# PaddlePaddle/Anakin

Measured on AMD Instinct MI355X. Metric: ResNet50 INT8 images/sec + p50 latency @ batch 1/8, 1×MI355X, higher is better.
Workload: dtype int8

## Files before the change

anakin_amd/build.py:

```python
import os
import subprocess
import sys

HERE = os.path.dirname(os.path.abspath(__file__))
CSRC = os.path.join(HERE, "csrc")
LIB = os.path.join(HERE, "libsaber_mi355x.so")
SOURCES = ["conv_igemm.hip", "elementwise.hip", "fc_small.hip", "conv1x1_chain.hip", "conv_chain_coop.hip", "conv_stage_coop.hip", "stage_xcd.hip", "conv1x1_gpool.hip", "conv3x3_b3h.hip", "conv1x1_pw.hip", "conv1x1_pwk.hip", "conv_stem_f32.hip", "fc_f32_splitk.hip", "conv_dw3x3.hip", "conv_group3x3.hip", "conv_sep.hip", "conv_ir.hip", "conv_fire.hip", "deconv.hip"] + \
    ["api_%s.hip" % n for n in ("conv", "select", "autotune", "ops", "chain", "sep", "ir", "fire", "deconv", "stage", "net", "net_optimize", "net_autotune", "capture", "gemm", "streams")] + \
    ["igemm_m%d_e%d.hip" % me for me in [(0, 0), (0, 1), (0, 2), (0, 3), (0, 4), (1, 0), (1, 1), (1, 2), (1, 3), (2, 3), (3, 3)]] + \
    ["igemm_dma_m%d_e%d.hip" % me for me in [(0, 0), (0, 1), (0, 2), (0, 3), (0, 4), (2, 3)]] + \
    ["halo_e%d.hip" % e for e in range(4)] + ["img_e%d.hip" % e for e in (0, 1, 3)] + ["stem_e%d.hip" % e for e in range(4)] + ["stem_pool.hip"]
FLAGS = ["--offload-arch=gfx950", "-O3", "-std=c++17", "-fPIC", "-ffp-contract=off", "-fno-fast-math",
         "-Wno-unused-result", "-mllvm", "-amdgpu-mfma-vgpr-form"]


def _stale(obj, deps):
    if not os.path.exists(obj):
        return True
    t = os.path.getmtime(obj)
    return any(os.path.getmtime(d) > t for d in deps)


def build(force=False, verbose=False):
    hipcc = os.environ.get("HIPCC", "/opt/rocm/bin/hipcc")
    objdir = os.path.join(HERE, "build")
    os.makedirs(objdir, exist_ok=True)
    import glob
    headers = sorted(glob.glob(os.path.join(CSRC, "*.h"))) + [os.path.join(HERE, "..", "include", "saber_hip.h")]
    objs = []
    procs = []
    for src in SOURCES:
        sp = os.path.join(CSRC, src)
        obj = os.path.join(objdir, src.replace(".hip", ".o"))
        objs.append(obj)
        deps = [h for h in headers if src.startswith("api_") or os.path.basename(h) != "api_internal.h"]
        if force or _stale(obj, [sp] + deps):
            cmd = [hipcc] + FLAGS + ["-c", sp, "-o", obj]
            if verbose:
                print(" ".join(cmd))
            procs.append((src, subprocess.Popen(cmd)))
# ... 35 lines not shown
```

anakin_amd/csrc/api_chain.hip:

```cpp
#include "api_internal.h"

enum : unsigned { CK_1X1 = 1, CK_3X3 = 2, CK_HEAD = 4, CK_PAIR = 8, CK_LED = CK_3X3 | CK_HEAD, CK_ANY = 15 };
static unsigned chain_kind(const saber_hip_chain* ch) { return !ch->c3 ? CK_1X1 : (ch->b2 ? CK_PAIR : (ch->b ? CK_3X3 : CK_HEAD)); }
static const struct { int c1; unsigned kinds; ChainForm f; } chain_forms[] = {
    {64, CK_ANY,            {4, 4, 4, 1, 1, CS_BASE, false}},
    {64, CK_ANY,            {2, 2, 4, 1, 1, CS_BASE, false}},
    {128, CK_1X1 | CK_LED,  {2, 2, 4, 1, 1, CS_BASE, false}},
    {128, CK_1X1 | CK_LED,  {1, 1, 4, 1, 1, CS_BASE, false}},
    {128, CK_1X1 | CK_LED,  {6, 2, 8, 1, 1, CS_W8, false}},
    {128, CK_1X1 | CK_LED,  {5, 1, 8, 1, 1, CS_W8, false}},
    {256, CK_1X1 | CK_LED,  {1, 1, 4, 1, 1, CS_BASE, false}},
    {256, CK_1X1,           {9, 1, 4, 2, 1, CS_SPLIT, false}},
    {256, CK_1X1,           {11, 1, 8, 2, 1, CS_SPLIT8, false}},
    {256, CK_LED,           {3, 1, 8, 1, 1, CS_W8, false}},
    {256, CK_3X3,           {7, 1, 8, 1, 2, CS_COOP2, true}},
    {256, CK_3X3,           {15, 2, 8, 1, 4, CS_COOP4, true}},
    {512, CK_1X1,           {1, 1, 4, 1, 1, CS_BASE, false}},
    {512, CK_1X1,           {9, 1, 4, 2, 1, CS_SPLIT, false}},
};
static void for_each_chain_form(const saber_hip_chain* ch, const std::function<void(const ChainForm&)>& fn) {
    for (const auto& r : chain_forms)
        if (r.c1 == ch->c1 && (r.kinds & chain_kind(ch))) fn(r.f);
}
static ChainForm chain_form_where(const saber_hip_chain* ch, const std::function<bool(const ChainForm& row, const ChainForm& found)>& take) {
    ChainForm f;
    for_each_chain_form(ch, [&](const ChainForm& c) { if (take(c, f)) f = c; });
    return f;
}
ChainForm chain_form(const saber_hip_chain* ch, int code) { return chain_form_where(ch, [&](const ChainForm& c, const ChainForm&) { return c.code == code; }); }
ChainForm chain_form_default(const saber_hip_chain* ch) { return chain_form_where(ch, [](const ChainForm&, const ChainForm& f) { return !f.code; }); }
ChainForm chain_form_plain(const saber_hip_chain* ch) { return chain_form_where(ch, [](const ChainForm& c, const ChainForm&) { return !c.placement; }); }
bool chain_form_valid(const saber_hip_chain* ch, int code) {
    const ChainForm f = chain_form(ch, code);
    return f.code && ch->d_stream[f.stream].p && (f.coop != 4 || ch->stage1);
}
std::string chain_form_name(const saber_hip_chain* ch) {
    const ChainForm& f = ch->form;
    const std::string c = std::to_string(ch->c1), w8 = f.waves == 8 && f.coop == 1 ? "_w8" : "";
    if (!ch->c3) return "chain1x1_c" + c + "_px" + std::to_string(16 * f.rows) + (f.split == 2 ? "_split2" : "") + w8;
    return std::string("conv3x3+") + (ch->b2 ? "conv1x1+pair1x1_c" : (ch->b ? "chain1x1_c" : "conv1x1_c")) + c + "_" + std::to_string(f.rows) + "x16" + w8 +
           (f.coop == 2 ? "_coop2" : "") + (f.coop == 4 ? "_coop4" : "");
}
void for_each_chain_candidate(const saber_hip_chain* ch, bool shared_device, const std::function<void(const ChainForm&)>& fn) {
    for_each_chain_form(ch, [&](const ChainForm& c) { if (!(shared_device && c.placement) && chain_form_valid(ch, c.code)) fn(c); });
}

static bool chain_1x1(const saber_hip_conv* o, bool sub_res_ok = false) {
    const saber_hip_conv_desc& d = o->d;
    return o->is_i8 && o->weights_set && !o->gpool && o->algo == ALGO_IGEMM_I8 && o->epi == EPI_I8_CONV && d.kh == 1 && d.kw == 1 &&
           d.stride_h == 1 && d.stride_w == 1 && d.pad_h == 0 && d.pad_w == 0 && d.group == 1 && !o->pair_k2 &&
           !o->pool_fused && !o->pool2 && !o->pre_quant && !o->pre_pad && o->c_eff == d.c && d.act_negative_slope == 0.f &&
           d.in_layout == SABER_HIP_NHWC && d.out_layout == SABER_HIP_NHWC && (d.res_stride <= 1 || sub_res_ok);
}
static void pack_chain_params(const saber_hip_conv* o, size_t chunks_pad, std::vector<uint8_t>& out) {
    const int K = o->d.k;
    out.assign(chunks_pad * 16, 0);
    for (int k4 = 0; k4 < K / 4; ++k4) {
        float* f = (float*)(out.data() + (size_t)k4 * 48);
        int* ip = (int*)(out.data() + (size_t)k4 * 48 + 32);
        for (int r = 0; r < 4; ++r) {
            const int k = k4 * 4 + r;
            f[r] = o->scale_host.empty() ? 1.f : o->scale_host[k];
            f[4 + r] = (o->has_bias && !o->bias_p_host.empty()) ? o->bias_p_host[k] : 0.f;
            ip[r] = o->comp_host.empty() ? 0 : o->comp_host[k];
        }
    }
}
// ... 471 lines not shown
        if (rc != SABER_HIP_OK) {
            delete ch;
            return rc;
        }
    }
    *out = ch;
    return SABER_HIP_OK;
}
int saber_hip_conv2d_chain_create(saber_hip_conv_t* a, saber_hip_conv_t* b, saber_hip_chain_t** out) {
    if (!b) return fail(SABER_HIP_INVALID_VALUE, "null argument");
    return chain_build(nullptr, a, b, out);
}
int saber_hip_conv2d_chain_create3(saber_hip_conv_t* conv3x3, saber_hip_conv_t* a, saber_hip_conv_t* b, saber_hip_chain_t** out) {
    if (!conv3x3) return fail(SABER_HIP_INVALID_VALUE, "null argument");
    return chain_build(conv3x3, a, b, out);
}
int saber_hip_conv2d_chain_create3_pair(saber_hip_conv_t* conv3x3, saber_hip_conv_t* a, saber_hip_conv_t* pair_a, saber_hip_conv_t* pair_b,
                                        saber_hip_chain_t** out) {
    if (!conv3x3 || !pair_a || !pair_b) return fail(SABER_HIP_INVALID_VALUE, "null argument");
    return chain_build(conv3x3, a, pair_a, out, pair_b);
}
void saber_hip_conv2d_chain_destroy(saber_hip_chain_t* ch) { delete ch; }
int saber_hip_conv2d_chain_set_tile(saber_hip_chain_t* ch, int tn) {
    if (!ch) return fail(SABER_HIP_INVALID_VALUE, "null argument");
    if (!chain_form_valid(ch, tn)) return fail(SABER_HIP_INVALID_VALUE, "chain: no kernel form with that code for this chain");
    ch->form = chain_form(ch, tn);
    return SABER_HIP_OK;
}
int saber_hip_conv2d_chain_get_tile(const saber_hip_chain_t* ch) { return ch ? ch->form.code : 0; }
int saber_hip_conv2d_chain_run(saber_hip_chain_t* ch, const void* x, const void* res, void* y_a, void* y_b,
                               saber_hip_stream_t stream) {
    return saber_hip_conv2d_chain_run3(ch, x, res, y_a, y_b, nullptr, stream);
}
int saber_hip_conv2d_chain_run3(saber_hip_chain_t* ch, const void* x, const void* res, void* y_a, void* y_b, void* y_c,
                                saber_hip_stream_t stream) {
    if (g_capture) return capture_unsupported("saber_hip_conv2d_chain_run (saber_hip_net_optimize forms chains itself)");
    if (!ch || !x || !res || !y_a || (ch->b && !y_b) || (ch->b2 && !y_c)) return fail(SABER_HIP_INVALID_VALUE, "null argument");
    const saber_hip_conv *a = ch->a, *b = ch->b;
    ChainKArgs k;
    std::memset(&k, 0, sizeof k);
    k.x = x; k.res = res;
    const ChainForm f = ch->form;
    k.wstream = ch->d_stream[f.stream].p;
    k.prm1 = ch->d_prm1.p;
    k.prm2 = ch->d_prm2.p;
    k.y1 = y_a; k.y2 = y_b;
    k.M = a->d.n * a->oh * a->ow;
    k.in_u8 = a->x_dtype == DT_U8;
    k.relu1 = a->d.act == SABER_HIP_ACT_RELU;
    k.res_relu = a->d.res_act == SABER_HIP_ACT_RELU;
    k.coeff_conv = a->d.coeff_conv; k.scale_conv = ch->scale_conv; k.coeff_res = a->d.coeff_res; k.scale_res = a->d.scale_res;
    if (b) {
        k.relu2 = b->d.act == SABER_HIP_ACT_RELU;
        k.out_u8_2 = b->d.out_dtype == SABER_HIP_U8;
    }
    if (ch->b2) {
        k.y2b = y_c;
        k.k2_split = b->d.k;
        k.relu2b = ch->b2->d.act == SABER_HIP_ACT_RELU;
        k.out_u8_2b = ch->b2->d.out_dtype == SABER_HIP_U8;
    }
    if (ch->c3) {
        k.prm0 = ch->d_prm0.p;
        k.zero = zero_page();
        if (!k.zero) return fail(SABER_HIP_RUNTIME_ERROR, "chain: zero page");
        k.N = a->d.n; k.H = a->d.h; k.W = a->d.w;
        k.tiles_x = (k.W + 15) / 16;
        k.tiles_per_img = k.tiles_x * ((k.H + f.rows - 1) / f.rows);
        k.mg_tiles_x = div_magic(k.tiles_x);
        k.mg_tpi = div_magic(k.tiles_per_img);
        k.in0_u8 = ch->c3->x_dtype == DT_U8;
        k.relu0 = ch->c3->d.act == SABER_HIP_ACT_RELU;
        k.s0 = ch->c3->d.stride_h;
        k.H0 = ch->c3->d.h; k.W0 = ch->c3->d.w;
        if (a->d.res_stride > 1) { k.res_sub = a->d.res_stride; k.res_H = a->d.res_h; k.res_W = a->d.res_w; }
    }
    if (f.coop == 4) {
        const int rc = stage_run(ch->stage1, x, res, &y_a, &y_b, (hipStream_t)stream);
        if (rc != SABER_HIP_OK) ch->form = chain_form_plain(ch);
        return rc;
    }
    if (f.coop == 2) {
        if (*(volatile unsigned*)ch->h_coop_err) {
            *(volatile unsigned*)ch->h_coop_err = 0u;
            ch->form = chain_form_plain(ch);
            return fail(SABER_HIP_RUNTIME_ERROR, "cooperative chain: an earlier launch's workgroup pairs did not share an XCD or timed out at their "
                        "barrier (its outputs are not valid); the chain now runs the single-workgroup form");
        }
        const CoopKArgs ck{k, ch->d_coop_ctr.p, ch->d_coop_xch.p, ch->d_coop_xcc.p, ch->h_coop_err, ch->coop_tiles};
        HIP_TRY(launch_conv_chain_coop(ck, (hipStream_t)stream));
        return SABER_HIP_OK;
    }
    HIP_TRY(launch_conv1x1_chain(k, ch->c1, ch->k1, ch->k2, f.rows, f.waves, f.split, ch->c3 ? 1 : 0, (hipStream_t)stream));
    return SABER_HIP_OK;
}
```

anakin_amd/csrc/api_internal.h:

```cpp
#pragma once
#include "../../include/saber_hip.h"
#include "kernels.h"

#include <cmath>
#include <cstdio>
#include <algorithm>
#include <cstdlib>
#include <cstring>
#include <functional>
#include <memory>
#include <mutex>
#include <string>
#include <utility>
#include <type_traits>
#include <vector>

using namespace saber_mi355x;

namespace saber_api {

extern thread_local std::string g_err;
inline int fail(int code, const std::string& msg) {
    g_err = msg;
    return code;
// ... 147 lines not shown
    bool has_bias = false, has_comp = false;
    std::string algo_name;
    int pair_k1 = 0, pair_k2 = 0, pair_relu2 = 0, pair_dtype2 = 0;
    const saber_hip_conv* pair_src_a = nullptr;
    const saber_hip_conv* pair_src_b = nullptr;
};

struct saber_hip_stem_pair {
    saber_hip_conv* stem = nullptr;
    const saber_hip_conv* a = nullptr;
    const saber_hip_conv* b = nullptr;
    DevBuf<uint8_t> d_w, d_prm;
};

enum ChainStream { CS_BASE, CS_SPLIT, CS_SPLIT8, CS_W8, CS_COOP2, CS_COOP4, CS_COUNT };
struct ChainForm {
    int code = 0;
    int rows = 0;
    int waves = 4;
    int split = 1;
    int coop = 1;
    ChainStream stream = CS_BASE;
    bool placement = false;
};

struct saber_hip_chain {
    saber_hip_conv* c3 = nullptr;
    saber_hip_conv* a = nullptr;
    saber_hip_conv* b = nullptr;
    saber_hip_conv* b2 = nullptr;
    int c1 = 0, k1 = 0, k2 = 0;
    float scale_conv = 1.f;
    std::vector<int8_t> tail_w3, tail_wa;
    ChainForm form;
    DevBuf<uint8_t> d_stream[CS_COUNT];
    DevBuf<uint8_t> d_prm0, d_prm1, d_prm2;
    DevBuf<uint8_t> d_coop_xch;
    DevBuf<uint8_t> d_stream_stage1;
    DevBuf<unsigned long long> d_coop_ctr;
    DevBuf<unsigned> d_coop_xcc;
    unsigned* h_coop_err = nullptr;
    int coop_tiles = 0;
    struct saber_hip_chain_stage* stage1 = nullptr;
    ~saber_hip_chain();
};

struct saber_hip_chain_stage {
    std::vector<saber_hip_chain*> chains;
    saber_hip_chain* tail = nullptr;
    DevBuf<uint8_t> d_tail_stream;
    const saber_hip_conv* head_a = nullptr;
    const saber_hip_conv* head_b = nullptr;
    DevBuf<uint8_t> d_head_stream, d_head_prm1, d_head_prm2;
    DevBuf<saber_mi355x::StageBlk> d_blk;
    DevBuf<unsigned long long> d_grp_ctr, d_img_ctr;
    DevBuf<uint8_t> d_xch;
    DevBuf<unsigned> d_xcc;
    unsigned* h_err = nullptr;
    int c1 = 0, n = 0, h = 0, w = 0, tiles_x = 0, tiles_per_img = 0;
    bool per_image = false;
    ~saber_hip_chain_stage() {
        if (h_err) (void)hipHostFree(h_err);
    }
};

struct saber_hip_sep {
// ... 112 lines not shown
        owner = true;
        return hipSuccess;
    }
    ~ColdScope() {
        if (owner) g_cold = nullptr;
    }
};

}

namespace saber_api {
enum OpKind { OP_CONV, OP_CONV_PAIR, OP_FC, OP_QUANT, OP_DEQUANT, OP_TRANSPOSE_IN, OP_ELT_I8, OP_ELT_F32, OP_POOL_I8, OP_POOL_F32, OP_POOL_F32_I8, OP_FC_Q, OP_SOFTMAX, OP_RELU_F32, OP_ACT_F32, OP_CONCAT, OP_DECONV };
enum Launch { LAUNCH_NONE, LAUNCH_OWN, LAUNCH_CHAIN, LAUNCH_CHAIN3, LAUNCH_STAGE, LAUNCH_STEM_PAIR, LAUNCH_SEP, LAUNCH_IR, LAUNCH_FIRE };
struct NetOp {
    OpKind kind;
    std::string name;
    saber_hip_conv* conv = nullptr;
    saber_hip_fc* fc = nullptr;
    saber_hip_deconv* deconv = nullptr;
    int in = -1, in2 = -1, out = -1, out2 = -1;
    std::vector<int> ins, cat_c;
    std::vector<float> cat_m;
    Launch launch = LAUNCH_OWN;
    int absorbed_by = -1;
    bool skip = false;
    std::string res_note;
    saber_hip_chain* chain = nullptr;
    int chain_out = -1;
    bool chain_on = false;
    saber_hip_chain* chain3 = nullptr;
    int chain3_res = -1, chain3_y1 = -1, chain3_y2 = -1;
    int chain3_y3 = -1;
    bool led_on = false;
    saber_hip_chain_stage* stage = nullptr;
    int stage_n = 0;
    bool stage_on = false;
    bool stage_name_kept = false;
    bool tail_on = false;
    int tail_of = -1;
    bool head_on = false;
    int head_of = -1;
    bool stage_y1_private = false;
    saber_hip_stem_pair* stem_pair = nullptr;
    int stem_y1 = -1, stem_y2 = -1;
    saber_hip_sep* sep = nullptr;
    int sep_out = -1;
    bool sep_on = false;
    saber_hip_ir* ir = nullptr;
    int ir_out = -1;
    bool ir_on = false;
    saber_hip_fire* fire = nullptr;
    int fire_out = -1;
    bool fire_on = false;
    int lane = 0;
    bool record = false;
    int p[16] = {0};
    float f[6] = {0};
    size_t count = 0;
};
template <typename F>
inline void op_for_each_input(const NetOp& o, F&& f) {
    if (o.kind == OP_CONCAT) {
        for (int t : o.ins) f(t);
        return;
    }
    if (o.in >= 0) f(o.in);
// ... 58 lines not shown
int sel_set(saber_hip_conv* op, const saber_api::ConvSel& s);
void sel_release_unused(saber_hip_conv* op);
void sel_name(saber_hip_conv* op);
unsigned long long sel_kernel_key(const saber_hip_conv* op, const saber_api::ConvSel& s);
int sel_launch(saber_hip_conv* op, saber_mi355x::ConvKArgs& a, hipStream_t s);
void for_each_candidate(const saber_hip_conv* op, const saber_api::ConvSel* best, const std::function<void(const saber_api::ConvSel&)>& fn);
bool dw_ok(const saber_hip_conv* op);
bool group_ok(const saber_hip_conv* op);
bool stem_ok(const saber_hip_conv* op);
bool fc_small_ok(const saber_hip_conv* op);
bool b3_tile_ok(const saber_hip_conv* op, int tile, int ks);
int dw_static_form(const saber_hip_conv* op);
int group_static_form(const saber_hip_conv* op);
constexpr long DW_STRIP_MIN_LANES = 150000;
void conv_fill_args(const saber_hip_conv* op, saber_mi355x::ConvKArgs& a, const void* x, void* y, const void* res);
int stem_pool_args(const saber_hip_conv* op, const void* x, void* y, void* workspace, hipStream_t s, saber_mi355x::ConvKArgs* a);
bool xcd_round_robin();
int split_prepare(saber_hip_conv* op);
bool img_conv_ok(const saber_hip_conv* op);
int img_conv_prepare(saber_hip_conv* op);
int pw_prepare(saber_hip_conv* op);
bool pw_eligible(const saber_hip_conv* op);
int img_conv_run(saber_hip_conv* op, const void* x, void* y, const void* res, void* y_pool, hipStream_t stream);
void img_conv_release(saber_hip_conv* op);
int net_launch(saber_hip_net* net, const NetOp& o, hipStream_t s);
bool fc_softmax_ok(const saber_hip_fc* fc, bool quantised_input = false);
int fc_run_softmax(saber_hip_fc* fc, const void* x, float* y, float* prob, void* workspace, hipStream_t s, bool quantised_input);
int fc_softmax_prepare(saber_hip_fc* fc);
int concat_check(int n_inputs, const int* channels, const float* mult, int dtype, int* row_bytes);
void net_resolve(saber_hip_net* net);
void net_drop_graph(saber_hip_net* net);
void net_set_chain_mode(saber_hip_net* net, int ia, int mode);
int net_chain_mode(const saber_hip_net* net, int ia);
void net_set_stage(saber_hip_net* net, int i0, bool on);
void net_set_head(saber_hip_net* net, int i0, bool on);
void net_set_tail(saber_hip_net* net, int i0, bool on);
ChainForm chain_form(const saber_hip_chain* ch, int code);
bool chain_form_valid(const saber_hip_chain* ch, int code);
ChainForm chain_form_default(const saber_hip_chain* ch);
ChainForm chain_form_plain(const saber_hip_chain* ch);
std::string chain_form_name(const saber_hip_chain* ch);
void for_each_chain_candidate(const saber_hip_chain* ch, bool shared_device, const std::function<void(const ChainForm&)>& fn);
bool conv_sep_ok(const saber_hip_conv* dw, const saber_hip_conv* pw, std::string* why);
bool sep_form_valid(const saber_hip_sep* sp, int code);
void for_each_sep_form(const saber_hip_sep* sp, const std::function<void(int code)>& fn);
int sep_static_form(const saber_hip_sep* sp);
void net_set_sep(saber_hip_net* net, int i, int code);
bool conv_ir_ok(const saber_hip_conv* expand, const saber_hip_conv* dw, const saber_hip_conv* project, std::string* why);
bool ir_form_valid(const saber_hip_ir* ir, int code);
void for_each_ir_form(const saber_hip_ir* ir, const std::function<void(int code)>& fn);
int ir_static_form(const saber_hip_ir* ir);
void net_set_ir(saber_hip_net* net, int i, int code);
bool conv_fire_ok(const saber_hip_conv* squeeze, const saber_hip_conv* e1, const saber_hip_conv* e3, std::string* why);
bool fire_form_valid(const saber_hip_fire* fr, int code);
void for_each_fire_form(const saber_hip_fire* fr, const std::function<void(int code)>& fn);
int fire_static_form(const saber_hip_fire* fr);
void net_set_fire(saber_hip_net* net, int i, int code);
bool deconv_form_valid(const saber_hip_deconv* op, int form);
int deconv_static_form(const saber_hip_deconv* op);
void for_each_deconv_form(const saber_hip_deconv* op, const std::function<void(int form)>& fn);
int stage_run(saber_hip_chain_stage* st, const void* x, const void* res, void* const* y1, void* const* y2, hipStream_t s, void* y_tail = nullptr,
              void* y_head = nullptr);
```

anakin_amd/csrc/api_net.hip:

```cpp
#include "api_internal.h"

#include <atomic>
static std::atomic<int> g_coop_fallbacks_total{0};

void net_drop_graph(saber_hip_net* net) {
    if (net->exec) (void)hipGraphExecDestroy(net->exec);
    if (net->graph) (void)hipGraphDestroy(net->graph);
    net->exec = nullptr;
    net->graph = nullptr;
}
int net_launch(saber_hip_net* net, const NetOp& o, hipStream_t s) {
    auto T = [&](int id) -> void* { return net->ptr(id); };
    void* ws = net->arena + net->ws_off;
    switch (o.kind) {
    case OP_CONV:
        switch (o.launch) {
        case LAUNCH_NONE: return SABER_HIP_OK;
        case LAUNCH_STAGE: {
            void* y1[saber_mi355x::STAGE4_LONG];
            void* y2[saber_mi355x::STAGE4_LONG];
            const NetOp* ops = &o;
            for (int k = 0; k < o.stage_n; ++k) {
                y1[k] = ops[3 * k].stage_y1_private ? nullptr : T(ops[3 * k].chain3_y1);
                y2[k] = T(ops[3 * k].chain3_y2);
            }
            void* const y_tail = o.tail_on ? T(ops[3 * o.stage_n].chain3_y1) : nullptr;
            const int rc = o.head_on ? stage_run(o.stage, T(ops[-1].in), nullptr, y1, y2, s, y_tail, T(o.in))
                                     : stage_run(o.stage, T(o.in), T(o.chain3_res), y1, y2, s, y_tail);
            if (rc == SABER_HIP_RUNTIME_ERROR) {
                ++net->coop_fallbacks;
                ++g_coop_fallbacks_total;
                net_set_stage(net, (int)(&o - net->ops.data()), false);
                net_drop_graph(net);
            }
            return rc;
        }
        case LAUNCH_STEM_PAIR: return saber_hip_conv2d_stem_pair_run(o.stem_pair, T(o.in), nullptr, T(o.stem_y1), T(o.stem_y2), ws, s);
        case LAUNCH_CHAIN3: {
            const int rc = saber_hip_conv2d_chain_run3(o.chain3, T(o.in), T(o.chain3_res), T(o.chain3_y1), T(o.chain3_y2), T(o.chain3_y3), s);
            if (rc == SABER_HIP_RUNTIME_ERROR) {
                ++net->coop_fallbacks;
                ++g_coop_fallbacks_total;
            }
            return rc;
        }
        case LAUNCH_CHAIN: return saber_hip_conv2d_chain_run(o.chain, T(o.in), T(o.in2), T(o.out), T(o.chain_out), s);
        case LAUNCH_SEP: return saber_hip_conv2d_sep_run(o.sep, T(o.in), nullptr, T(o.sep_out), s);
        case LAUNCH_IR: return saber_hip_conv2d_ir_run(o.ir, T(o.in), nullptr, nullptr, T(o.ir_out), s);
        case LAUNCH_FIRE: return saber_hip_conv2d_fire_run(o.fire, T(o.in), nullptr, T(o.fire_out), s);
        case LAUNCH_OWN: break;
        }
        if (o.conv->gpool) return saber_hip_conv2d_run_gpool(o.conv, T(o.in), T(o.out), T(o.in2), T(o.out2), s);
        return saber_hip_conv2d_run(o.conv, T(o.in), T(o.out), T(o.in2), ws, s);
    case OP_CONV_PAIR:
        if (o.skip) return SABER_HIP_OK;
        return saber_hip_conv2d_run_pair(o.conv, T(o.in), T(o.out), T(o.out2), s);
    case OP_FC:
        if (o.out2 >= 0) return fc_run_softmax(o.fc, T(o.in), (float*)T(o.out), (float*)T(o.out2), ws, s, false);
        return saber_hip_fc_run(o.fc, T(o.in), (float*)T(o.out), ws, s);
    case OP_QUANT:
        return saber_hip_quantize_nchw_to_nhwc(o.p[0], o.p[1], o.p[2], o.p[3], o.p[4], o.p[5], o.f[0],
                                               (const float*)T(o.in), T(o.out), s);
    case OP_DEQUANT:
        return saber_hip_dequantize_nhwc_to_nchw(o.p[0], o.p[1], o.p[2], o.p[3], o.p[4], o.f[0], T(o.in),
                                                 (float*)T(o.out), s);
    case OP_TRANSPOSE_IN:
        return saber_hip_transpose_nchw_to_nhwc_f32(o.p[0], o.p[1], o.p[2], o.p[3], o.p[4], (const float*)T(o.in),
                                                    (float*)T(o.out), s);
    case OP_ELT_I8:
        return saber_hip_eltwise_sum_i8(o.count, (const int8_t*)T(o.in), (const int8_t*)T(o.in2), o.f[0], o.f[1],
                                        o.f[2], o.f[3], o.p[0], (int8_t*)T(o.out), s);
// ... 231 lines not shown
    net->ws_off = off;
    off += (net->ws_bytes + 255) / 256 * 256;
    net->arena_bytes = off ? off : 256;
    HIP_TRY(hipMalloc((void**)&net->arena, net->arena_bytes));
    HIP_TRY(hipMemset(net->arena, 0, net->arena_bytes));
    HIP_TRY(hipStreamSynchronize(nullptr));
    net->finalized = true;
    return SABER_HIP_OK;
}
int saber_hip_net_compact_arena(saber_hip_net_t* net, const int* keep, int n_keep) {
    if (!net || !net->finalized) return fail(SABER_HIP_INVALID_VALUE, "compact_arena: net not finalized");
    const int nt = (int)net->tensor_bytes.size(), nops = (int)net->ops.size();
    for (const NetOp& o : net->ops)
        if (o.lane) return SABER_HIP_OK;
    std::vector<int> first(nt, nops), last(nt, -1), writes(nt, 0), reads(nt, 0);
    std::vector<char> pinned(nt, 0);
    for (int i = 0; i < n_keep; ++i)
        if (keep && keep[i] >= 0 && keep[i] < nt) pinned[keep[i]] = 1;
    std::vector<int> g_lo(nops), g_hi(nops);
    for (int i = 0; i < nops; ++i) g_lo[i] = g_hi[i] = i;
    auto span = [&](int i, int n) {
        const int hi = std::min(nops - 1, i + n - 1);
        int lo = i;
        for (int j = i; j <= hi; ++j) lo = std::min(lo, g_lo[j]);
        int h2 = hi;
        for (int j = i; j <= hi; ++j) h2 = std::max(h2, g_hi[j]);
        for (int j = lo; j <= h2; ++j) { g_lo[j] = std::min(g_lo[j], lo); g_hi[j] = std::max(g_hi[j], h2); }
    };
    for (int i = 0; i < nops; ++i) {
        const NetOp& o = net->ops[i];
        if (o.stage) span(i, 3 * o.stage_n + (o.stage->tail ? 2 : 0));
        if (o.stage && o.stage->head_a && i > 0) span(i - 1, 2);
        if (o.chain3) span(i, 3);
        if (o.chain) span(i, 2);
        if (o.stem_pair) span(i, 2);
        if (o.sep) span(i, 2);
        if (o.fire) span(i, 4);
        if (o.ir) span(i, 3);
        if ((o.kind == OP_FC || o.kind == OP_FC_Q) && o.out2 >= 0) span(i, 2);
    }
    for (int i = 0; i < nops; ++i) {
        const NetOp& o = net->ops[i];
        const int rd[] = {o.in, o.in2, o.chain3_res};
        const int wr[] = {o.out, o.out2, o.chain_out, o.chain3_y1, o.chain3_y2, o.chain3_y3, o.stem_y1, o.stem_y2, o.sep_out, o.ir_out, o.fire_out};
        auto touch = [&](int t) {
            if (t < 0 || t >= nt) return;
            first[t] = std::min(first[t], g_lo[i]);
            last[t] = std::max(last[t], g_hi[i]);
        };
        for (int t : rd) { touch(t); if (t >= 0 && t < nt) ++reads[t]; }
        for (size_t k = 1; k < o.ins.size(); ++k) { touch(o.ins[k]); if (o.ins[k] >= 0 && o.ins[k] < nt) ++reads[o.ins[k]]; }
        for (int t : wr) { touch(t); if (t >= 0 && t < nt) ++writes[t]; }
    }
    for (int t = 0; t < nt; ++t)
        if (net->tensor_ext[t] || !writes[t] || !reads[t] || last[t] < 0) pinned[t] = 1;
    for (int t = 0; t < nt; ++t)
        if (pinned[t]) { first[t] = -1; last[t] = nops; }
    std::vector<int> order;
    for (int t = 0; t < nt; ++t)
        if (!net->tensor_ext[t]) order.push_back(t);
    auto slot = [&](int t) { return (net->tensor_bytes[t] + 255) / 256 * 256; };
    std::stable_sort(order.begin(), order.end(), [&](int a, int b) { return slot(a) > slot(b); });
    std::vector<size_t> off(nt, 0);
    std::vector<int> placed;
    size_t top = 0;
    for (int t : order) {
// ... 12 lines not shown
        top = std::max(top, at + sz);
        placed.push_back(t);
    }
    const size_t ws_off = top, total = std::max<size_t>(256, top + (net->ws_bytes + 255) / 256 * 256);
    if (total >= net->arena_bytes) return SABER_HIP_OK;
    char* fresh = nullptr;
    HIP_TRY(hipMalloc((void**)&fresh, total));
    HIP_TRY(hipMemset(fresh, 0, total));
    HIP_TRY(hipDeviceSynchronize());
    for (int t = 0; t < nt; ++t)
        if (!net->tensor_ext[t] && !writes[t] && net->tensor_bytes[t])
            HIP_TRY(hipMemcpy(fresh + off[t], net->arena + net->tensor_off[t], net->tensor_bytes[t], hipMemcpyDeviceToDevice));
    HIP_TRY(hipDeviceSynchronize());
    (void)hipFree(net->arena);
    net->arena = fresh;
    net->arena_bytes = total;
    net->ws_off = ws_off;
    for (int t = 0; t < nt; ++t)
        if (!net->tensor_ext[t]) net->tensor_off[t] = off[t];
    net->compacted = true;
    net_drop_graph(net);
    return SABER_HIP_OK;
}
int saber_hip_net_arena_compacted(const saber_hip_net_t* net) { return net && net->compacted ? 1 : 0; }
void* saber_hip_net_tensor_ptr(saber_hip_net_t* net, int id) {
    if (!net->finalized || id < 0 || id >= (int)net->tensor_off.size()) return nullptr;
    return net->ptr(id);
}
size_t saber_hip_net_arena_bytes(const saber_hip_net_t* net) { return net->arena_bytes; }
int saber_hip_net_num_ops(const saber_hip_net_t* net) { return (int)net->ops.size(); }
const char* saber_hip_net_op_name(const saber_hip_net_t* net, int i) {
    return (i >= 0 && i < (int)net->ops.size()) ? net->ops[i].name.c_str() : "";
}
static int net_prepare_lanes(saber_hip_net* net) {
    if (net->lanes_ready) return SABER_HIP_OK;
    const int nops = (int)net->ops.size();
    net->writer.assign(net->tensor_bytes.size(), -1);
    net->ev_op.assign(nops, nullptr);
    net->has_side = false;
    std::vector<int> w(net->tensor_bytes.size(), -1);
    std::vector<std::vector<int>> rd(net->tensor_bytes.size());
    for (int i = 0; i < nops; ++i) {
        NetOp& o = net->ops[i];
        if (o.lane) net->has_side = true;
        int ins[1 + CONCAT_MAX_INPUTS] = {o.out}, n_ins = 1;
        op_for_each_input(o, [&](int t) { ins[n_ins++] = t; });
        for (int k = 0; k < n_ins; ++k) {
            const int t = ins[k];
            if (t >= 0 && w[t] >= 0 && net->ops[w[t]].lane != o.lane) net->ops[w[t]].record = true;
        }
        const int outs[2] = {o.out, o.out2};
        for (int t : outs) {
            if (t < 0) continue;
            for (int r : rd[t])
                if (net->ops[r].lane != o.lane) net->ops[r].record = true;
            rd[t].clear();
            w[t] = i;
        }
        op_for_each_input(o, [&](int t) { rd[t].push_back(i); });
    }
    if (net->has_side) {
        HIP_TRY(hipStreamCreateWithFlags(&net->side, hipStreamNonBlocking));
        HIP_TRY(hipEventCreateWithFlags(&net->ev_start, hipEventDisableTiming));
        HIP_TRY(hipEventCreateWithFlags(&net->ev_join, hipEventDisableTiming));
        for (int i = 0; i < nops; ++i)
            if (net->ops[i].record) HIP_TRY(hipEventCreateWithFlags(&net->ev_op[i], hipEventDisableTiming));
    }
    net->lanes_ready = true;
    return SABER_HIP_OK;
}

int saber_hip_net_run(saber_hip_net_t* net, saber_hip_stream_t stream) {
    if (!net->finalized) return fail(SABER_HIP_INVALID_VALUE, "net not finalized");
    int rc = net_prepare_lanes(net);
    if (rc) return rc;
    hipStream_t main_s = (hipStream_t)stream;
    if (!net->has_side) {
        for (const NetOp& o : net->ops) {
            rc = net_launch(net, o, main_s);
            if (rc) return rc;
        }
        return SABER_HIP_OK;
    }
    HIP_TRY(hipEventRecord(net->ev_start, main_s));
    HIP_TRY(hipStreamWaitEvent(net->side, net->ev_start, 0));
    std::fill(net->writer.begin(), net->writer.end(), -1);
    std::vector<std::vector<int>> readers(net->tensor_bytes.size());
    bool side_dirty = false;
    for (size_t i = 0; i < net->ops.size(); ++i) {
        const NetOp& o = net->ops[i];
        hipStream_t s = o.lane ? net->side : main_s;
        int ins[1 + CONCAT_MAX_INPUTS] = {o.out}, n_ins = 1;
        op_for_each_input(o, [&](int t) { ins[n_ins++] = t; });
        for (int k = 0; k < n_ins; ++k) {
            const int t = ins[k];
            if (t < 0) continue;
            const int wi = net->writer[t];
            if (wi >= 0 && net->ops[wi].lane != o.lane) HIP_TRY(hipStreamWaitEvent(s, net->ev_op[wi], 0));
        }
        const int outs[2] = {o.out, o.out2};
        for (int t : outs) {
            if (t < 0) continue;
            for (int r : readers[t])
                if (net->ops[r].lane != o.lane) HIP_TRY(hipStreamWaitEvent(s, net->ev_op[r], 0));
            readers[t].clear();
        }
        rc = net_launch(net, o, s);
        if (rc) return rc;
        if (o.record) HIP_TRY(hipEventRecord(net->ev_op[i], s));
        if (o.lane) side_dirty = true;
        net->writer[o.out] = (int)i;
        if (o.out2 >= 0) net->writer[o.out2] = (int)i;
        op_for_each_input(o, [&](int t) { readers[t].push_back((int)i); });
    }
    if (side_dirty) {
        HIP_TRY(hipEventRecord(net->ev_join, net->side));
        HIP_TRY(hipStreamWaitEvent(main_s, net->ev_join, 0));
    }
    return SABER_HIP_OK;
}
int saber_hip_net_set_lane(saber_hip_net_t* net, int index, int lane) {
    if (index < 0 || index >= (int)net->ops.size() || lane < 0 || lane > 1) return fail(SABER_HIP_INVALID_VALUE, "bad op index / lane");
    if (net->lanes_ready) return fail(SABER_HIP_INVALID_VALUE, "lanes are fixed after the first run");
    for (const NetOp& o : net->ops)
        if (lane && (o.chain || o.chain3 || o.stem_pair || o.sep || o.ir || o.fire))
            return fail(SABER_HIP_INVALID_VALUE, "the net has launches that span several ops' tensors (conv1x1 chains, the stem pair, separable sites): lanes must be assigned before saber_hip_net_optimize");
    if (lane) {
        const NetOp& o = net->ops[index];
        const size_t ws = o.kind == OP_CONV && o.conv ? o.conv->ws_bytes : (o.kind == OP_FC && o.fc ? saber_hip_fc_workspace_bytes(o.fc) : 0);
        if (ws) return fail(SABER_HIP_INVALID_VALUE, "an op that needs the shared workspace cannot run on the side lane");
    }
    net->ops[index].lane = lane;
    return SABER_HIP_OK;
}
int saber_hip_net_run_op(saber_hip_net_t* net, int index, saber_hip_stream_t stream) {
    if (!net->finalized || index < 0 || index >= (int)net->ops.size()) return fail(SABER_HIP_INVALID_VALUE, "bad op index");
    return net_launch(net, net->ops[index], (hipStream_t)stream);
}
static bool net_coop_error_pending(const saber_hip_net* net) {
    for (const NetOp& o : net->ops) {
        if (o.stage && o.stage->h_err && *(volatile unsigned*)o.stage->h_err) return true;
        if (const saber_hip_chain* ch = o.chain3)
            if ((ch->h_coop_err && *(volatile unsigned*)ch->h_coop_err) || (ch->stage1 && ch->stage1->h_err && *(volatile unsigned*)ch->stage1->h_err))
                return true;
    }
    return false;
// ... 10 lines not shown
    if (rc != SABER_HIP_OK) net_drop_graph(net);
    return rc;
}
int saber_hip_net_replay(saber_hip_net_t* net, saber_hip_stream_t stream) {
    if (!net->exec) return fail(SABER_HIP_INVALID_VALUE, "net not captured");
    if (net_coop_error_pending(net)) return saber_hip_net_status(net);
    HIP_TRY(hipGraphLaunch(net->exec, (hipStream_t)stream));
    return SABER_HIP_OK;
}
int saber_hip_net_coop_fallbacks(const saber_hip_net_t* net) { return net ? net->coop_fallbacks : 0; }
int saber_hip_coop_fallbacks_total(void) { return g_coop_fallbacks_total.load(); }
static void conv_work(const saber_hip_conv* c, double& bytes, double& flops) {
    const saber_hip_conv_desc& d = c->d;
    const double esz_in = d.in_dtype == SABER_HIP_F32 ? 4 : 1, esz_out = d.out_dtype == SABER_HIP_F32 ? 4 : 1;
    const double esz_w = c->is_i8 ? 1 : 4;
    const double in_el = (double)d.n * d.h * d.w * d.c;
    const int oh = c->oh, ow = c->ow;
    const double out_el = (double)d.n * ((c->pool_fused || c->pool2) ? c->pool_oh * c->pool_ow : oh * ow) * d.k;
    bytes += in_el * esz_in + out_el * esz_out + (double)d.k * (d.c / d.group) * d.kh * d.kw * esz_w;
    if (d.res_mode != SABER_HIP_RES_NONE) bytes += (double)d.n * oh * ow * d.k * esz_out;
    flops += 2.0 * d.n * oh * ow * (double)d.k * (d.c / d.group) * d.kh * d.kw;
}
int saber_hip_net_op_work(const saber_hip_net_t* net, int index, double* bytes, double* flops) {
    if (!net || index < 0 || index >= (int)net->ops.size() || !bytes || !flops) return fail(SABER_HIP_INVALID_VALUE, "bad argument");
    *bytes = 0; *flops = 0;
    const NetOp& o = net->ops[index];
    auto tb = [&](int t) { return t >= 0 ? (double)net->tensor_bytes[t] : 0.0; };
    switch (o.kind) {
    case OP_CONV:
        if (o.skip) return SABER_HIP_OK;
        conv_work(o.conv, *bytes, *flops);
        for (int j = index + 1; j < (int)net->ops.size(); ++j)
            if (net->ops[j].absorbed_by == index && net->ops[j].conv) conv_work(net->ops[j].conv, *bytes, *flops);
        return SABER_HIP_OK;
    case OP_CONV_PAIR:
        if (!o.skip) conv_work(o.conv, *bytes, *flops);
        return SABER_HIP_OK;
    case OP_FC:
    case OP_FC_Q: {
        const saber_hip_fc_desc& d = o.fc->d;
        const double esz = d.int8_weights ? 1 : 4;
        *bytes = (double)d.m * d.k * (o.kind == OP_FC_Q || d.in_dtype != SABER_HIP_F32 ? 1 : 4) + (double)d.m * d.n * 4 + (double)d.n * d.k * esz;
        *flops = 2.0 * d.m * d.n * d.k;
        if (o.out2 >= 0) *bytes += 2.0 * tb(o.out2);
        return SABER_HIP_OK;
    }
    case OP_DECONV: {
        const saber_hip_conv_desc& d = o.deconv->d;
        const double wel = (double)d.c * (d.k / d.group) * d.kh * d.kw;
        *bytes = 4.0 * ((double)d.n * d.h * d.w * d.c + (double)d.n * o.deconv->oh * o.deconv->ow * d.k + wel);
        *flops = 2.0 * d.n * d.h * d.w * wel;
        return SABER_HIP_OK;
    }
    default:
        if (o.skip) return SABER_HIP_OK;
        *bytes = tb(o.out) + tb(o.out2);
        op_for_each_input(o, [&](int t) { *bytes += tb(t); });
        return SABER_HIP_OK;
    }
}
int saber_hip_net_time_pass(saber_hip_net_t* net, saber_hip_stream_t stream, int iters, float* out_us) {
    if (!net || !net->finalized || iters <= 0 || !out_us) return fail(SABER_HIP_INVALID_VALUE, "bad argument");
    hipStream_t s = (hipStream_t)stream;
    const size_t n = net->ops.size();
    struct Events {
        std::vector<hipEvent_t> v;
// ... 51 lines not shown
        HIP_TRY(hipEventElapsedTime(&ms, evp.e0, evp.e1));
        if (it) acc += ms;
    }
    *out_us = (float)(acc * 1000.0 / iters);
    return SABER_HIP_OK;
}
int saber_hip_net_time_ops(saber_hip_net_t* net, saber_hip_stream_t stream, int iters, float* out_us) {
    hipStream_t s = (hipStream_t)stream;
    EventPair evp;
    HIP_TRY(evp.init());
    hipEvent_t e0 = evp.e0, e1 = evp.e1;
    for (size_t i = 0; i < net->ops.size(); ++i) {
        int rc = net_launch(net, net->ops[i], s);
        if (rc) return rc;
        HIP_TRY(hipEventRecord(e0, s));
        for (int it = 0; it < iters; ++it) net_launch(net, net->ops[i], s);
        HIP_TRY(hipEventRecord(e1, s));
        HIP_TRY(hipEventSynchronize(e1));
        float ms = 0;
        HIP_TRY(hipEventElapsedTime(&ms, e0, e1));
        out_us[i] = ms * 1000.f / iters;
    }
    return SABER_HIP_OK;
}
int saber_hip_net_tensor_unwritten(const saber_hip_net_t* net, int id) {
    if (id < 0 || id >= (int)net->tensor_bytes.size()) return 0;
    if (net->tensor_bytes[id] == 0) return 1;
    for (const NetOp& o : net->ops) {
        const Launch by = o.skip ? net->ops[o.absorbed_by].launch : o.launch;
        if (o.out == id && (o.launch == LAUNCH_CHAIN3 || o.launch == LAUNCH_STEM_PAIR || o.launch == LAUNCH_SEP || (o.chain3 && by == LAUNCH_STAGE))) return 1;
        if (o.out == id && (o.launch == LAUNCH_IR || (o.skip && by == LAUNCH_IR && (int)(&o - net->ops.data()) == o.absorbed_by + 1))) return 1;
        if (o.out == id && o.kind == OP_CONV && (o.launch == LAUNCH_FIRE || (o.skip && by == LAUNCH_FIRE))) return 1;
        if (o.launch == LAUNCH_STAGE && o.head_on && o.chain3_res == id) return 1;
        if (o.chain3 && o.stage_y1_private && o.chain3_y1 == id && (o.launch == LAUNCH_STAGE || (o.skip && by == LAUNCH_STAGE))) return 1;
    }
    return 0;
}
int saber_hip_net_status(saber_hip_net_t* net) {
    if (!net || !net->finalized) return fail(SABER_HIP_INVALID_VALUE, "net not finalized");
    int bad = 0;
    for (size_t i = 0; i < net->ops.size(); ++i) {
        NetOp& o = net->ops[i];
        if (o.stage && o.stage->h_err && *(volatile unsigned*)o.stage->h_err) {
            *(volatile unsigned*)o.stage->h_err = 0u;
            if (o.stage_on) net_set_stage(net, (int)i, false);
            ++bad;
        }
        saber_hip_chain* ch = o.chain3;
        if (ch) {
            unsigned* words[2] = {ch->h_coop_err, ch->stage1 ? ch->stage1->h_err : nullptr};
            for (unsigned* w : words)
                if (w && *(volatile unsigned*)w) {
                    *(volatile unsigned*)w = 0u;
                    if (ch->form.placement) ch->form = chain_form_plain(ch);
                    ++bad;
                }
        }
    }
    if (!bad) return SABER_HIP_OK;
    net->coop_fallbacks += bad;
    g_coop_fallbacks_total += bad;
    net_resolve(net);
    net_drop_graph(net);
    return fail(SABER_HIP_RUNTIME_ERROR, "a cooperative launch of the last pass did not complete (workgroups on different XCDs, or a hand-off "
                "timed out: another kernel held the CUs); its outputs are not valid - those sites now launch block by block: run the pass again");
}
// ... 40 lines not shown
```

anakin_amd/csrc/api_net_autotune.hip:

```cpp
#include "api_internal.h"

static saber_hip_conv* net_op_conv(saber_hip_net* net, int index) {
    if (index < 0 || index >= (int)net->ops.size()) return nullptr;
    NetOp& o = net->ops[index];
    if (o.kind == OP_CONV || o.kind == OP_CONV_PAIR) return o.conv;
    if (o.kind == OP_FC || o.kind == OP_FC_Q) return o.fc ? o.fc->conv : nullptr;
    return nullptr;
}
int saber_hip_net_get_choice(saber_hip_net_t* net, int index) {
    if (net && index >= 0 && index < (int)net->ops.size() && net->ops[index].kind == OP_DECONV)
        return (18 << 16) | saber_hip_deconv2d_get_tile(net->ops[index].deconv);
    saber_hip_conv* c = net_op_conv(net, index);
    int choice = (c && !c->pool_fused && (c->algo <= ALGO_IGEMM_F32 || dw_ok(c) || group_ok(c))) ? saber_hip_conv2d_get_tile(c) : 0;
    if (!c) return choice;
    const NetOp& o = net->ops[index];
    if (o.chain) choice |= (1 << 28) | ((o.chain_on ? o.chain->form.code : 0) << 24);
    if (o.chain3) choice |= (1 << 29) | ((o.led_on ? o.chain3->form.code : 0) << 24);
    if (o.sep) choice |= (3 << 28) | ((o.sep_on ? o.sep->form : 0) << 24);
    if (o.ir) choice |= (int)0x80000000u | ((o.ir_on ? o.ir->form : 0) << 24);
    if (o.fire) choice |= (int)0x80000000u | ((o.fire_on ? o.fire->form : 0) << 24);
    if (o.stage && o.stage_on) choice |= 1 << 30;
    if (o.stage && o.stage_on && o.tail_on) choice |= (int)0x80000000u;
    if (o.head_of >= 0 && net->ops[o.head_of].stage_on && net->ops[o.head_of].head_on) choice |= 1 << 29;
    return choice;
}
int saber_hip_net_stage_blocks(const saber_hip_net_t* net, int index) {
    if (!net || index < 0 || index >= (int)net->ops.size()) return 0;
    const NetOp& o = net->ops[index];
    return o.stage ? (o.stage->c1 == 64 ? -o.stage_n : o.stage_n) : 0;
}
int saber_hip_net_stage_head(const saber_hip_net_t* net, int index) {
    if (!net || index < 1 || index >= (int)net->ops.size() || !net->ops[index].stage) return -1;
    return net->ops[index - 1].head_of == index ? index - 1 : -1;
}
int saber_hip_net_set_choice(saber_hip_net_t* net, int index, int choice) {
    if (net && index >= 0 && index < (int)net->ops.size() && net->ops[index].kind == OP_DECONV) {
        if (net->reproducible_fp32 || ((choice >> 16) & 0xff) != 18) return SABER_HIP_OK;
        const int rc = saber_hip_deconv2d_set_tile(net->ops[index].deconv, choice & 0xffff);
        if (rc) return rc;
        net_resolve(net);
        net_drop_graph(net);
        return SABER_HIP_OK;
    }
    saber_hip_conv* c = net_op_conv(net, index);
    const bool ir_bits = c && net->ops[index].ir && ((unsigned)choice >> 30) == 2u;
    const int ir_tn = (choice >> 24) & 15;
    if (ir_bits && ir_tn && !ir_form_valid(net->ops[index].ir, ir_tn)) return saber_hip_conv2d_ir_set_tile(net->ops[index].ir, ir_tn);
    const bool fire_bits = c && net->ops[index].fire && ((unsigned)choice >> 30) == 2u;
    if (fire_bits && ir_tn && !fire_form_valid(net->ops[index].fire, ir_tn)) return saber_hip_conv2d_fire_set_tile(net->ops[index].fire, ir_tn);
    if (fire_bits && !(choice & 0xffffff)) {
        net_set_fire(net, index, ir_tn);
        net_drop_graph(net);
        return SABER_HIP_OK;
    }
    if (ir_bits && !(choice & 0xffffff)) {
        net_set_ir(net, index, ir_tn);
        net_drop_graph(net);
        return SABER_HIP_OK;
    }
    if (!c || !choice || c->pool_fused || (c->algo > ALGO_IGEMM_F32 && !dw_ok(c) && !group_ok(c))) return SABER_HIP_OK;
    if (net->reproducible_fp32 && !c->is_i8) return SABER_HIP_OK;
    if (net->ops[index].kind == OP_CONV_PAIR && index > 0 && net->ops[index - 1].stem_pair) return SABER_HIP_OK;
    const int chain_bits = (choice >> 24) & 63;
    const bool stage_on = ((choice >> 30) & 1) && !net->shared_device;
    const bool tail_on = stage_on && (((unsigned)choice >> 31) & 1u);
    choice &= 0xffffff;
    if (net->shared_device && ((choice >> 16) & 0xff) == 11) choice &= ~(0xf << 12);
    NetOp& o = net->ops[index];
    saber_hip_chain* ch = index + 1 >= (int)net->ops.size() ? nullptr : ((o.chain3 && (chain_bits & 32)) ? o.chain3 : ((o.chain && (chain_bits & 16)) ? o.chain : nullptr));
    int tn = chain_bits & 15;
    if (ch && net->shared_device && chain_form(ch, tn).placement) tn = chain_form_plain(ch).code;
    if (ch && tn && !chain_form_valid(ch, tn)) return saber_hip_conv2d_chain_set_tile(ch, tn);
    const bool sep_bits = o.sep && (chain_bits & 48) == 48;
    if (sep_bits && tn && !sep_form_valid(o.sep, tn)) return saber_hip_conv2d_sep_set_tile(o.sep, tn);
    int rc = choice ? saber_hip_conv2d_set_tile(c, choice) : SABER_HIP_OK;
    if (rc) return rc;
    o.res_note.clear();
    o.stage_name_kept = false;
    if (ch && tn) (void)saber_hip_conv2d_chain_set_tile(ch, tn);
    const bool in_stage = o.chain3 && o.skip && !o.stage && o.tail_of < 0;
    const int mode = ch ? net_chain_mode(net, ch == o.chain3 ? index + 1 : index) : 0;
    if (ch && ch == o.chain3) net_set_chain_mode(net, index + 1, (tn || in_stage) ? 2 : std::min(mode, 1));
    else if (ch) net_set_chain_mode(net, index, mode == 2 ? 2 : (tn ? 1 : 0));
    if (o.stage) net_set_stage(net, index, stage_on);
    if (o.stage) net_set_tail(net, index, tail_on);
    if (o.head_of >= 0) net_set_head(net, o.head_of, (chain_bits & 32) && !net->shared_device);
    if (sep_bits) net_set_sep(net, index, tn);
    if (ir_bits) net_set_ir(net, index, ir_tn);
    if (fire_bits) net_set_fire(net, index, ir_tn);
    net_resolve(net);
    net_drop_graph(net);
    return SABER_HIP_OK;
}

static int net_consolidate_kernels(saber_hip_net* net, hipStream_t s) {
    if (net->has_side) return SABER_HIP_OK;
    if (const char* e = std::getenv("SABER_HIP_NO_CONSOLIDATE"))
        if (e[0] == '1') return SABER_HIP_OK;
    struct Site { int op; unsigned long long key; ConvSel choice; };
    auto conv_of = [&](const NetOp& o) -> saber_hip_conv* {
        if (o.launch != LAUNCH_OWN) return nullptr;
        if (o.kind != OP_CONV && o.kind != OP_CONV_PAIR) return nullptr;
        if (net->reproducible_fp32 && o.conv && !o.conv->is_i8) return nullptr;
        return (o.conv && !o.conv->pool_fused && o.conv->algo <= ALGO_IGEMM_F32) ? o.conv : nullptr;
    };
    auto collect = [&]() {
        std::vector<Site> v;
        for (int i = 0; i < (int)net->ops.size(); ++i)
            if (saber_hip_conv* c = conv_of(net->ops[i])) v.push_back({i, sel_kernel_key(c, c->sel), c->sel});
        return v;
    };
    EventPair ev;
    HIP_TRY(ev.init());
    auto forward_ms = [&](float* ms) -> int {
        int rc = 0;
        for (int i = 0; i < 3 && !rc; ++i) rc = saber_hip_net_run(net, s);
        if (rc) return rc;
        HIP_TRY(hipEventRecord(ev.e0, s));
        for (int i = 0; i < 30 && !rc; ++i) rc = saber_hip_net_run(net, s);
// ... 90 lines not shown
            if (saber_hip_deconv2d_set_tile(o.deconv, form) != SABER_HIP_OK) return;
            if (time_enqueued(s, run, 20, &us) != SABER_HIP_OK) return;
            if (best_form < 0 || us < best) { best = us; best_form = form; }
        });
        if (best_form < 0) return fail(SABER_HIP_RUNTIME_ERROR, "autotune: no form of a deconv op could be timed");
        int rc = saber_hip_deconv2d_set_tile(o.deconv, best_form);
        if (!rc) rc = run();
        if (rc) return rc;
    }
    net_resolve(net);
    const char* log_env = std::getenv("SABER_HIP_AUTOTUNE_LOG");
    const bool log_cands = g_cold && log_env && log_env[0] == '1';
    auto log_cand = [&](const saber_hip_conv* c, const std::string& name, float t) {
        if (log_cands) std::fprintf(stderr, "autotune [%dx%dx%d c%d k%d %dx%d] %-40s %8.2f us\n", c->d.n, c->d.h, c->d.w, c->d.c, c->d.k, c->d.kh, c->d.kw, name.c_str(), t);
    };
    for (size_t i = 0; i < net->ops.size(); ++i)
        if (net->ops[i].stage) net_set_stage(net, (int)i, false);
    for (size_t i = 0; i < net->ops.size(); ++i) {
        NetOp& A = net->ops[i];
        const int ia = (int)i;
        NetOp* H = (ia > 0 && net->ops[ia - 1].chain3) ? &net->ops[ia - 1] : nullptr;
        if (!A.chain && !H) continue;
        const int first = H ? ia - 1 : ia;
        const int last = (A.chain || (H && H->chain3->b2)) ? ia + 1 : ia;
        hipStream_t s = (hipStream_t)stream;
        auto run_all = [&]() -> int {
            int rc = 0;
            for (int k = first; k <= last; ++k) rc |= net_launch(net, net->ops[k], s);
            return rc;
        };
        auto timed = [&](float* t) { return time_enqueued(s, run_all, 20, t); };
        float best = 0.f;
        int best_mode = 0, best_tn = 0;
        net_set_chain_mode(net, ia, 0);
        int rc = timed(&best);
        if (rc) return rc;
        log_cand(A.conv, "separate", best);
        for (int mode = A.chain ? 1 : 2; mode <= (H ? 2 : 1); ++mode) {
            saber_hip_chain* ch = mode == 2 ? H->chain3 : A.chain;
            for_each_chain_candidate(ch, net->shared_device, [&](const ChainForm& f) {
                float ms = -1.f;
                if (saber_hip_conv2d_chain_set_tile(ch, f.code) != SABER_HIP_OK) return;
                net_set_chain_mode(net, ia, mode);
                const int rt = timed(&ms);
                log_cand(A.conv, (mode == 2 ? H->name : A.name).substr(5), ms);
                if (rt == SABER_HIP_OK && ms < best) { best = ms; best_mode = mode; best_tn = f.code; }
            });
        }
        if (best_mode) (void)saber_hip_conv2d_chain_set_tile(best_mode == 2 ? H->chain3 : A.chain, best_tn);
        net_set_chain_mode(net, ia, best_mode);
        rc = run_all();
        if (rc) return rc;
    }
    for (size_t i = 0; i < net->ops.size(); ++i) {
        NetOp& H0 = net->ops[i];
        if (!H0.stage || net->shared_device) continue;
        const bool has_tail = H0.stage->tail != nullptr;
        const bool has_head = saber_hip_net_stage_head(net, (int)i) >= 0;
        const int first = (int)i, last = first + 3 * H0.stage_n - 1 + (has_tail ? 2 : 0);
        hipStream_t s = (hipStream_t)stream;
        auto run_all = [&]() -> int {
            int rc = 0;
            for (int k = first - (has_head ? 1 : 0); k <= last; ++k) rc |= net_launch(net, net->ops[k], s);
            return rc;
        };
        auto timed = [&](float* t) { return time_enqueued(s, run_all, 20, t); };
        std::vector<int> modes(H0.stage_n), tns(H0.stage_n);
        for (int k = 0; k < H0.stage_n; ++k) {
            modes[k] = net_chain_mode(net, first + 3 * k + 1);
            tns[k] = net->ops[first + 3 * k].chain3->form.code;
        }
        float sep = 0.f, one = 0.f;
        int rc = timed(&sep);
        if (rc) return rc;
        log_cand(H0.conv, "separate", sep);
        net_set_stage(net, first, true);
        net_set_tail(net, first, false);
        bool ok = timed(&one) == SABER_HIP_OK && hipStreamSynchronize(s) == hipSuccess && !*(volatile unsigned*)H0.stage->h_err;
        log_cand(H0.conv, H0.name.substr(5), ok ? one : -1.f);
        if (ok && has_tail) {
            float wt = 0.f;
            net_set_tail(net, first, true);
            const bool ok_t = timed(&wt) == SABER_HIP_OK && hipStreamSynchronize(s) == hipSuccess && !*(volatile unsigned*)H0.stage->h_err;
            log_cand(H0.conv, H0.name.substr(5), ok_t ? wt : -1.f);
            if (*(volatile unsigned*)H0.stage->h_err) ok = false;
            else if (ok_t && wt < one) one = wt;
            else net_set_tail(net, first, false);
        }
        if (ok && one < sep && has_head) {
            float wh = 0.f;
            net_set_head(net, first, true);
            const bool ok_h = timed(&wh) == SABER_HIP_OK && hipStreamSynchronize(s) == hipSuccess && !*(volatile unsigned*)H0.stage->h_err;
            log_cand(H0.conv, H0.name.substr(5), ok_h ? wh : -1.f);
            if (*(volatile unsigned*)H0.stage->h_err) ok = false;
            else if (ok_h && wh < one * 0.99f) one = wh;
            else net_set_head(net, first, false);
// ... 88 lines not shown
```

anakin_amd/csrc/api_net_optimize.hip:

```cpp
#include "api_internal.h"

void net_resolve(saber_hip_net* net) {
    std::vector<NetOp>& ops = net->ops;
    const int n = (int)ops.size();
    enum { IN_CHAIN, IN_STAGE, IN_STEM, IN_SEP, IN_IR, IN_FIRE };
    static const char* const covered[] = {"conv:(in the chain launch)", "conv:(in the stage launch)", "conv:(in the stem launch)", "conv:(in the separable launch)",
                                          "conv:(in the inverted-residual launch)", "conv:(in the fire launch)"};
    std::vector<int> in(n, IN_CHAIN);
    for (NetOp& o : ops) {
        o.launch = LAUNCH_OWN;
        o.absorbed_by = -1;
    }
    auto absorb = [&](int j, int by, int what) {
        ops[j].launch = LAUNCH_NONE;
        ops[j].absorbed_by = by;
        in[j] = what;
    };
    for (int i = 0; i < n; ++i) {
        NetOp& o = ops[i];
        if (o.launch == LAUNCH_NONE) continue;
        if ((o.kind == OP_FC || o.kind == OP_FC_Q) && o.out2 >= 0) {
            for (int j = i + 1; j < n; ++j)
                if (ops[j].kind == OP_SOFTMAX && ops[j].out == o.out2) { absorb(j, i, IN_CHAIN); break; }
        }
        if (o.kind != OP_CONV || i + 1 >= n) continue;
        if (o.stage && o.stage_on) {
            o.launch = LAUNCH_STAGE;
            for (int k = 0; k < o.stage_n; ++k) {
                if (k) absorb(i + 3 * k, i, IN_STAGE);
                absorb(i + 3 * k + 1, i, IN_CHAIN);
                absorb(i + 3 * k + 2, i, IN_CHAIN);
            }
            if (o.tail_on)
                for (int j = i + 3 * o.stage_n; j < i + 3 * o.stage_n + 2; ++j) absorb(j, i, IN_STAGE);
            if (o.head_on) absorb(i - 1, i, IN_STAGE);
        } else if (o.stem_pair) {
            o.launch = LAUNCH_STEM_PAIR;
            absorb(i + 1, i, IN_STEM);
        } else if (o.chain3 && o.led_on) {
            o.launch = LAUNCH_CHAIN3;
            absorb(i + 1, i, IN_CHAIN);
            if (o.chain3->b || o.chain3->b2) absorb(i + 2, i, IN_CHAIN);
        } else if (o.chain && o.chain_on) {
            o.launch = LAUNCH_CHAIN;
            absorb(i + 1, i, IN_CHAIN);
        } else if (o.sep && o.sep_on) {
            o.launch = LAUNCH_SEP;
            absorb(i + 1, i, IN_SEP);
        } else if (o.ir && o.ir_on && i + 2 < n) {
            o.launch = LAUNCH_IR;
            absorb(i + 1, i, IN_IR);
            absorb(i + 2, i, IN_IR);
        } else if (o.fire && o.fire_on && i + 3 < n) {
            o.launch = LAUNCH_FIRE;
            for (int j = i + 1; j <= i + 3; ++j) absorb(j, i, IN_FIRE);
        }
    }
    for (int i = 0; i < n; ++i) {
        NetOp& o = ops[i];
        o.skip = o.launch == LAUNCH_NONE;
        if (o.kind == OP_CONCAT) {
            o.name = "concat" + std::to_string(o.ins.size()) + (o.skip ? " (in the fire launch)" : "");
        } else if (o.kind == OP_DECONV) {
            o.name = std::string("deconv:") + o.deconv->algo_name;
        } else if (o.kind == OP_SOFTMAX) {
            o.name = o.skip ? "softmax_f32 (in the fc launch)" : "softmax_f32";
        } else if (o.kind == OP_FC || o.kind == OP_FC_Q) {
            o.name = std::string("fc:") + o.fc->conv->algo_name;
            if (o.out2 >= 0) o.name += fc_softmax_ok(o.fc, o.kind == OP_FC_Q) ? "+softmax" : " | softmax_f32";
        } else if (o.kind == OP_CONV || o.kind == OP_CONV_PAIR) {
            const std::string own = o.conv->algo_name;
            const bool kept = o.stage_name_kept && !o.skip;
            switch (kept ? (o.stage ? LAUNCH_STAGE : LAUNCH_NONE) : o.launch) {
            case LAUNCH_NONE: o.name = covered[kept ? IN_STAGE : in[i]]; break;
            case LAUNCH_OWN: o.name = "conv:" + own + o.res_note; break;
            case LAUNCH_CHAIN: o.name = "conv:" + chain_form_name(o.chain); break;
            case LAUNCH_CHAIN3: o.name = "conv:" + chain_form_name(o.chain3); break;
            case LAUNCH_SEP: o.name = std::string("conv:") + saber_hip_conv2d_sep_algo(o.sep); break;
            case LAUNCH_IR: o.name = std::string("conv:") + saber_hip_conv2d_ir_algo(o.ir); break;
            case LAUNCH_FIRE: o.name = std::string("conv:") + saber_hip_conv2d_fire_algo(o.fire); break;
            case LAUNCH_STEM_PAIR: o.name = "conv:" + own + "+pair1x1_" + std::to_string(o.stem_pair->a->d.k) + "+" + std::to_string(o.stem_pair->b->d.k); break;
            case LAUNCH_STAGE:
                o.name = std::string(o.head_on && !kept ? "conv:[pair1x1]+stage_c" : "conv:stage_c") + std::to_string(o.stage->c1) + "_" + std::to_string(o.stage_n) + "x[conv3x3+chain1x1]_2x16" +
                         (o.stage->c1 == 256 ? "_coop4" : "") + (o.tail_on && !kept ? "+[conv3x3/2+conv1x1]" : "");
                break;
            }
        }
    }
}
void net_set_chain_mode(saber_hip_net* net, int ia, int mode) {
    NetOp& A = net->ops[ia];
    NetOp* H = (ia > 0 && net->ops[ia - 1].chain3) ? &net->ops[ia - 1] : nullptr;
    if (H) H->led_on = mode == 2;
    if (H) H->stage_name_kept = false;
    A.chain_on = A.chain && mode >= 1;
    A.res_note.clear();
    net_resolve(net);
}
int net_chain_mode(const saber_hip_net* net, int ia) {
    const NetOp& A = net->ops[ia];
    return (ia > 0 && net->ops[ia - 1].chain3 && net->ops[ia - 1].led_on) ? 2 : (A.chain_on ? 1 : 0);
}
void net_set_tail(saber_hip_net* net, int i0, bool on) {
    NetOp& H0 = net->ops[i0];
    if (!H0.stage || !H0.stage->tail) return;
    H0.tail_on = on;
    net_resolve(net);
}
void net_set_head(saber_hip_net* net, int i0, bool on) {
    NetOp& H0 = net->ops[i0];
    if (!H0.stage || !H0.stage->head_a || i0 < 1 || net->ops[i0 - 1].head_of != i0) return;
    H0.head_on = on;
    net_resolve(net);
}
void net_set_stage(saber_hip_net* net, int i0, bool on) {
    NetOp& H0 = net->ops[i0];
    if (!H0.stage) return;
    if (on || H0.stage_on)
        for (int k = 0; k < H0.stage_n; ++k) {
            net->ops[i0 + 3 * k].led_on = true;
            net->ops[i0 + 3 * k].stage_name_kept = !on;
            net->ops[i0 + 3 * k + 1].chain_on = net->ops[i0 + 3 * k + 1].chain != nullptr;
        }
    if (on) H0.tail_on = H0.stage->tail != nullptr;
    if (!on) H0.tail_on = H0.head_on = false;
    H0.stage_on = on;
    net_resolve(net);
}
void net_set_sep(saber_hip_net* net, int i, int code) {
    NetOp& D = net->ops[i];
    if (!D.sep || i + 1 >= (int)net->ops.size()) return;
    if (code && saber_hip_conv2d_sep_set_tile(D.sep, code) != SABER_HIP_OK) code = 0;
    D.sep_on = code != 0;
    net_resolve(net);
// ... 347 lines not shown
            D.sep = sp;
            D.sep_out = P.out;
            net_set_sep(net, (int)i, sep_static_form(sp));
            ++removed;
        }
    }
    if (flags & 16) {
        for (size_t i = 0; i + 1 < ops.size(); ++i) {
            NetOp& A = ops[i];
            NetOp& B = ops[i + 1];
            if (A.kind != OP_CONV || B.kind != OP_CONV || !A.conv || !B.conv || A.chain || A.skip || B.chain || A.lane || B.lane ||
                A.chain3 || B.chain3 || in_ir(A) || in_ir(B))
                continue;
            if (A.conv->d.res_mode != SABER_HIP_RES_ELTWISE || B.in != A.out || A.in2 < 0 || B.in2 >= 0) continue;
            saber_hip_chain* ch = nullptr;
            if (saber_hip_conv2d_chain_create(A.conv, B.conv, &ch) != SABER_HIP_OK) continue;
            net->owned_chains.push_back(ch);
            A.chain = ch;
            A.chain_out = B.out;
            net_set_chain_mode(net, (int)i, ch->c1 <= 256 ? 1 : 0);
            if (A.chain_on) ++removed;
        }
    }
    if (flags & 32) {
        for (size_t i = 0; i + 2 < ops.size(); ++i) {
            NetOp& Hd = ops[i];
            NetOp& A = ops[i + 1];
            NetOp& B = ops[i + 2];
            if (!A.chain || Hd.kind != OP_CONV || !Hd.conv || Hd.chain3 || Hd.chain || Hd.skip || Hd.lane || Hd.in2 >= 0 ||
                A.in != Hd.out)
                continue;
            if (readers(Hd.out) != 1) continue;
            saber_hip_chain* ch = nullptr;
            if (saber_hip_conv2d_chain_create3(Hd.conv, A.conv, B.conv, &ch) != SABER_HIP_OK) continue;
            net->owned_chains.push_back(ch);
            Hd.chain3 = ch;
            Hd.chain3_res = A.in2; Hd.chain3_y1 = A.out; Hd.chain3_y2 = B.out;
            const bool was = A.chain_on;
            net_set_chain_mode(net, (int)i + 1, ch->c1 <= 128 ? 2 : (was ? 1 : 0));
            if (Hd.led_on) removed += was ? 1 : 2;
        }
        for (size_t i = 0; i + 1 < ops.size(); ++i) {
            NetOp& Hd = ops[i];
            NetOp& A = ops[i + 1];
            if (A.chain || A.skip || A.kind != OP_CONV || !A.conv || A.conv->d.res_mode != SABER_HIP_RES_ELTWISE || A.in2 < 0 || A.lane ||
                Hd.kind != OP_CONV || !Hd.conv || Hd.chain3 || Hd.chain || Hd.skip || Hd.lane || Hd.in2 >= 0 || A.in != Hd.out || in_ir(Hd) || in_ir(A))
                continue;
            if (readers(Hd.out) != 1) continue;
            saber_hip_chain* ch = nullptr;
            NetOp* P = (flags & 1024) && i + 2 < ops.size() ? &ops[i + 2] : nullptr;
            if (P && (P->kind != OP_CONV_PAIR || P->lane || P->skip || P->in != A.out || !P->conv || !P->conv->pair_src_a || !P->conv->pair_src_b)) P = nullptr;
            if (P) {
                if (readers(A.out) != 1 || saber_hip_conv2d_chain_create3_pair(Hd.conv, A.conv, const_cast<saber_hip_conv*>(P->conv->pair_src_a),
                                                                   const_cast<saber_hip_conv*>(P->conv->pair_src_b), &ch) != SABER_HIP_OK)
                    P = nullptr;
            }
            if (!P && saber_hip_conv2d_chain_create3(Hd.conv, A.conv, nullptr, &ch) != SABER_HIP_OK) continue;
            net->owned_chains.push_back(ch);
            Hd.chain3 = ch;
            Hd.chain3_res = A.in2; Hd.chain3_y1 = A.out; Hd.chain3_y2 = P ? P->out : -1; Hd.chain3_y3 = P ? P->out2 : -1;
            net_set_chain_mode(net, (int)i + 1, ch->c1 <= 128 ? 2 : 0);
            if (Hd.led_on) removed += P ? 2 : 1;
        }
    }
    if ((flags & 256) && (flags & 32) && !two_lanes) {
        for (size_t i = 0; i + 2 < ops.size();) {
            auto block_ok = [&](size_t j) {
                return j + 2 < ops.size() && ops[j].chain3 && ops[j].chain3->b && !ops[j].stage && ops[j].chain3_y2 >= 0 &&
                       ((ops[j].chain3->c1 == 256 && ops[j].chain3->stage1) || ((ops[j].chain3->c1 == 128 || ops[j].chain3->c1 == 64) && ops[j].chain3->d_stream_stage1.p));
            };
            if (!block_ok(i)) { ++i; continue; }
            std::vector<saber_hip_chain*> run{ops[i].chain3};
            while ((int)run.size() < saber_mi355x::STAGE4_LONG) {
                const size_t p = i + 3 * (run.size() - 1), j = p + 3;
                if (!block_ok(j) || ops[j].chain3->c1 != run[0]->c1 || ops[j].in != ops[p].chain3_y2 || ops[j].chain3_res != ops[p].chain3_y1) break;
                run.push_back(ops[j].chain3);
            }
            if (run.size() >= 2) {
                saber_hip_chain_stage* st = nullptr;
                const size_t pl = i + 3 * (run.size() - 1), jt = pl + 3;
                saber_hip_chain* tail = nullptr;
                if (jt + 1 < ops.size() && run[0]->c1 == 256 && ops[jt].chain3 && !ops[jt].chain3->b && !ops[jt].chain3->b2 && !ops[jt].stage &&
                    ops[jt].chain3->c1 == 256 && ops[jt].chain3->c3->d.stride_h == 2 && ops[jt].in == ops[pl].chain3_y2 &&
                    ops[jt].chain3_res == ops[pl].chain3_y1 && ops[jt].chain3_y1 >= 0)
// ... 71 lines not shown
```

anakin_amd/csrc/kernels.h:

```cpp
#pragma once
#include <hip/hip_runtime.h>
#include <stddef.h>
#include <stdint.h>

#ifdef SABER_TIMELINE
extern __device__ unsigned long long* saber_tl_buf;
#define SABER_TL_DECL unsigned long long tl_[16] = {0, 0, 0, 0, 0, 0, 0, 0, 0, 0, 0, 0, 0, 0, 0, 0}
#define SABER_TL(i) tl_[i] = wall_clock64()
#define SABER_TL_FLUSH()                                                                   \
    do {                                                                                   \
        if (threadIdx.x == 0 && saber_tl_buf)                                              \
            for (int i_ = 0; i_ < 16; ++i_) saber_tl_buf[(size_t)blockIdx.x * 16 + i_] = tl_[i_]; \
    } while (0)
#else
#define SABER_TL_DECL do { } while (0)
#define SABER_TL(i) do { } while (0)
#define SABER_TL_FLUSH() do { } while (0)
#endif

namespace saber_mi355x {

enum { DT_F32 = 0, DT_S8 = 1, DT_U8 = 2 };

enum {
// ... 73 lines not shown
struct ChainKArgs {
    const void* x;
    const void* wstream;
    const void* res;
    const void* prm1;
    const void* prm2;
    void* y1;
    void* y2;
    int M, in_u8;
    int relu1, res_relu;
    float coeff_conv, scale_conv, coeff_res, scale_res;
    int relu2, out_u8_2;
    const void* prm0;
    const void* zero;
    int N, H, W;
    int tiles_x, tiles_per_img;
    unsigned mg_tiles_x, mg_tpi;
    int in0_u8, relu0;
    int s0, H0, W0;
    int res_sub, res_H, res_W;
    void* y2b;
    int k2_split, relu2b, out_u8_2b;
};
struct CoopKArgs {
    ChainKArgs c;
    unsigned long long* coop_ctr;
    void* coop_xch;
    unsigned* coop_xcc;
    unsigned* coop_err;
    int n_tiles;
};
bool conv1x1_chain_ok(int c1, int k1, int k2);
hipError_t launch_conv1x1_chain(const ChainKArgs& a, int c1, int k1, int k2, int rows, int waves, int split, int with3x3, hipStream_t s);
hipError_t launch_conv_chain_coop(const CoopKArgs& a, hipStream_t s);

struct StageBlk {
    const void* wstream;
    const void* prm0;
    const void* prm1;
    const void* prm2;
    float coeff_conv, scale_conv, coeff_res, scale_res;
    int in0_u8, relu0, in_u8, relu1, res_relu, relu2, out_u8_2, pad_;
};
template <int MAXB>
struct Stage4KArgs {
    const void* x;
    const void* res;
    const void* zero;
    const StageBlk* blk;
    unsigned long long* grp_ctr;
    unsigned long long* img_ctr;
    void* xch;
    unsigned* xcc;
    unsigned* err;
    int nblk, N, H, W;
    int tiles_x, tiles_per_img;
    unsigned mg_tiles_x, mg_tpi, mg_wpi;
    int per_image;
    void* y1[MAXB];
    void* y2[MAXB];
    void* head_y;
};
constexpr int STAGE4_SHORT = 8, STAGE4_LONG = 24;
hipError_t launch_conv_stage4(const Stage4KArgs<STAGE4_SHORT>& a, bool tail, bool head, hipStream_t s);
hipError_t launch_conv_stage4(const Stage4KArgs<STAGE4_LONG>& a, bool tail, bool head, hipStream_t s);
hipError_t launch_conv_stage1_c128(const Stage4KArgs<STAGE4_SHORT>& a, hipStream_t s);
// ... 250 lines not shown
```

anakin_amd/lib.py:

```python
import ctypes as C
import os

HERE = os.path.dirname(os.path.abspath(__file__))
LIB_PATH = os.environ.get("SABER_MI355X_LIB") or os.path.join(HERE, "libsaber_mi355x.so")

F32, S8, U8, S32 = 0, 1, 2, 3
NHWC, NCHW = 0, 1
ACT_NONE, ACT_RELU = 0, 1
POOL_MAX, POOL_AVG_INCL, POOL_AVG_EXCL = 0, 1, 2
RES_NONE, RES_SUM_INPLACE, RES_ELTWISE = 0, 1, 2
TILES = ["32x32", "64x32", "64x64", "128x64", "64x128", "128x128"]

SYMBOLS = [
    "saber_hip_last_error", "saber_hip_device_ok",
    "saber_hip_conv2d_create", "saber_hip_conv2d_set_weights", "saber_hip_conv2d_workspace_bytes",
    "saber_hip_conv2d_out_shape", "saber_hip_conv2d_run", "saber_hip_conv2d_destroy",
    "saber_hip_conv2d_get_quantized_weights", "saber_hip_conv2d_algo", "saber_hip_conv2d_set_tile",
    "saber_hip_conv2d_get_tile", "saber_hip_conv2d_autotune", "saber_hip_conv2d_set_pooling",
    "saber_hip_conv2d_create_pair", "saber_hip_conv2d_run_pair", "saber_hip_conv2d_autotune_pair",
    "saber_hip_net_add_conv_pair",
    "saber_hip_conv2d_chain_create", "saber_hip_conv2d_chain_create3", "saber_hip_conv2d_chain_create3_pair", "saber_hip_conv2d_chain_destroy", "saber_hip_conv2d_chain_run",
    "saber_hip_conv2d_chain_run3",
    "saber_hip_conv2d_chain_set_tile", "saber_hip_conv2d_chain_get_tile",
    "saber_hip_conv2d_stage_create", "saber_hip_conv2d_stage_destroy", "saber_hip_conv2d_stage_run", "saber_hip_conv2d_stage_create_tail", "saber_hip_conv2d_stage_run_tail",
    "saber_hip_conv2d_stage_create_head", "saber_hip_conv2d_stage_run_head",
    "saber_hip_conv2d_stem_pair_create", "saber_hip_conv2d_stem_pair_destroy", "saber_hip_conv2d_stem_pair_run",
    "saber_hip_conv2d_sep_create", "saber_hip_conv2d_sep_run", "saber_hip_conv2d_sep_set_tile", "saber_hip_conv2d_sep_get_tile",
    "saber_hip_conv2d_sep_algo", "saber_hip_conv2d_sep_destroy",
    "saber_hip_conv2d_ir_create", "saber_hip_conv2d_ir_run", "saber_hip_conv2d_ir_set_tile", "saber_hip_conv2d_ir_get_tile",
    "saber_hip_conv2d_ir_algo", "saber_hip_conv2d_ir_destroy",
    "saber_hip_conv2d_set_global_pooling", "saber_hip_conv2d_run_gpool",
    "saber_hip_stage_create", "saber_hip_stage_num_tensors", "saber_hip_stage_run", "saber_hip_stage_status", "saber_hip_stage_trace", "saber_hip_stage_destroy",
    "saber_hip_fc_create", "saber_hip_fc_set_weights", "saber_hip_fc_workspace_bytes", "saber_hip_fc_run",
    "saber_hip_fc_destroy", "saber_hip_fc_algo", "saber_hip_fc_set_tile", "saber_hip_gemm_f32", "saber_hip_gemm_f32_release_plans",
    "saber_hip_gemm_i8_create", "saber_hip_gemm_i8_workspace_bytes", "saber_hip_gemm_i8_run", "saber_hip_gemm_i8_destroy",
    "saber_hip_quantize_nchw_to_nhwc", "saber_hip_dequantize_nhwc_to_nchw",
    "saber_hip_transpose_nchw_to_nhwc_f32", "saber_hip_transpose_nhwc_to_nchw_f32",
    "saber_hip_quantize_flat_s8", "saber_hip_eltwise_sum_i8", "saber_hip_eltwise_sum_f32", "saber_hip_relu_f32", "saber_hip_activation_f32", "saber_hip_prelu_f32",
    "saber_hip_pool_out_dim", "saber_hip_pool_out_dim2", "saber_hip_pool2d_i8_nhwc", "saber_hip_pool2d_f32", "saber_hip_pool2d_f32_from_i8", "saber_hip_pool2d_f32_from_i8_q", "saber_hip_fc_run_q", "saber_hip_fc_run_softmax", "saber_hip_softmax_f32",
    "saber_hip_net_add_pool_f32_from_i8_q", "saber_hip_net_add_fc_q", "saber_hip_net_optimize", "saber_hip_net_num_launches", "saber_hip_net_tensor_unwritten", "saber_hip_net_get_choice", "saber_hip_net_set_choice", "saber_hip_net_stage_blocks", "saber_hip_net_stage_head", "saber_hip_net_time_op_in_pass", "saber_hip_net_status", "saber_hip_net_inject_coop_error", "saber_hip_net_coop_fallbacks", "saber_hip_coop_fallbacks_total",
    "saber_hip_net_create", "saber_hip_net_add_tensor", "saber_hip_net_add_conv", "saber_hip_net_add_fc",
    "saber_hip_net_add_quantize", "saber_hip_net_add_dequantize", "saber_hip_net_add_transpose_in_f32", "saber_hip_net_add_eltwise_i8",
    "saber_hip_net_add_eltwise_f32", "saber_hip_net_add_pool_i8", "saber_hip_net_add_pool_f32",
    "saber_hip_net_add_pool_f32_from_i8", "saber_hip_net_add_softmax", "saber_hip_net_set_lane", "saber_hip_net_finalize", "saber_hip_net_tensor_ptr",
    "saber_hip_net_arena_bytes", "saber_hip_net_num_ops", "saber_hip_net_run", "saber_hip_net_run_op",
    "saber_hip_net_capture", "saber_hip_net_replay", "saber_hip_net_time_ops", "saber_hip_net_time_pass", "saber_hip_net_op_work", "saber_hip_net_op_name",
    "saber_hip_net_autotune", "saber_hip_net_destroy",
    "saber_hip_net_add_relu_f32", "saber_hip_net_add_activation_f32", "saber_hip_net_bind_tensor", "saber_hip_net_num_tensors", "saber_hip_net_tensor_bytes",
    "saber_hip_capture_begin", "saber_hip_capture_end", "saber_hip_capture_active", "saber_hip_net_tensor_of_ptr",
    "saber_hip_net_compact_arena", "saber_hip_net_arena_compacted", "saber_hip_serving_streams",
    "saber_hip_concat_nhwc", "saber_hip_net_add_concat",
    "saber_hip_conv2d_fire_create", "saber_hip_conv2d_fire_run", "saber_hip_conv2d_fire_set_tile", "saber_hip_conv2d_fire_get_tile",
    "saber_hip_conv2d_fire_algo", "saber_hip_conv2d_fire_destroy",
    "saber_hip_deconv2d_create", "saber_hip_deconv2d_set_weights", "saber_hip_deconv2d_out_shape", "saber_hip_deconv2d_run",
    "saber_hip_deconv2d_algo", "saber_hip_deconv2d_set_tile", "saber_hip_deconv2d_get_tile", "saber_hip_deconv2d_destroy",
    "saber_hip_net_add_deconv",
]


class StagePhase(C.Structure):
    _fields_ = [("conv", C.c_void_p), ("in_", C.c_int), ("out", C.c_int), ("res", C.c_int)]


class ConvDesc(C.Structure):
    _fields_ = [(n, C.c_int) for n in
                ("n", "h", "w", "c", "k", "kh", "kw", "pad_h", "pad_w", "stride_h", "stride_w", "dil_h", "dil_w",
                 "group", "in_dtype", "out_dtype", "in_layout", "out_layout", "act", "res_mode", "res_act")] + \
               [("sum_scale", C.c_float), ("coeff_conv", C.c_float), ("coeff_res", C.c_float),
                ("scale_res", C.c_float), ("int8_weights", C.c_int), ("act_negative_slope", C.c_float),
                ("res_has_dtype", C.c_int), ("res_dtype", C.c_int), ("res_stride", C.c_int), ("res_h", C.c_int),
                ("res_w", C.c_int)]


# ... 22 lines not shown
            "(there is no CPU fallback for the MI355X Saber target)")
    lib = C.CDLL(LIB_PATH)
    P, I, F, Z = C.c_void_p, C.c_int, C.c_float, C.c_size_t
    lib.saber_hip_last_error.restype = C.c_char_p
    lib.saber_hip_conv2d_create.argtypes = [C.POINTER(ConvDesc), C.POINTER(P)]
    lib.saber_hip_conv2d_set_weights.argtypes = [P, P, I, P, P, F, F]
    lib.saber_hip_conv2d_workspace_bytes.argtypes = [P]
    lib.saber_hip_conv2d_workspace_bytes.restype = Z
    lib.saber_hip_conv2d_out_shape.argtypes = [P, C.POINTER(I), C.POINTER(I)]
    lib.saber_hip_conv2d_out_shape.restype = None
    lib.saber_hip_conv2d_run.argtypes = [P, P, P, P, P, P]
    lib.saber_hip_conv2d_destroy.argtypes = [P]
    lib.saber_hip_conv2d_destroy.restype = None
    lib.saber_hip_conv2d_get_quantized_weights.argtypes = [P, P, P]
    lib.saber_hip_conv2d_algo.argtypes = [P]
    lib.saber_hip_conv2d_algo.restype = C.c_char_p
    lib.saber_hip_conv2d_set_tile.argtypes = [P, I]
    lib.saber_hip_conv2d_get_tile.argtypes = [P]
    lib.saber_hip_conv2d_set_pooling.argtypes = [P] + [I] * 8
    lib.saber_hip_conv2d_autotune.argtypes = [P, P, P, P, P, P, I]
    lib.saber_hip_conv2d_create_pair.argtypes = [P, P, C.POINTER(P)]
    lib.saber_hip_conv2d_run_pair.argtypes = [P, P, P, P, P]
    lib.saber_hip_conv2d_autotune_pair.argtypes = [P, P, P, P, P, I]
    lib.saber_hip_net_add_conv_pair.argtypes = [P, P, I, I, I]
    lib.saber_hip_conv2d_chain_create.argtypes = [P, P, C.POINTER(P)]
    lib.saber_hip_conv2d_chain_create3.argtypes = [P, P, P, C.POINTER(P)]
    lib.saber_hip_net_tensor_unwritten.argtypes = [P, I]
    lib.saber_hip_net_num_launches.argtypes = [P]
    lib.saber_hip_conv2d_chain_destroy.argtypes = [P]
    lib.saber_hip_conv2d_chain_destroy.restype = None
    lib.saber_hip_conv2d_chain_run.argtypes = [P, P, P, P, P, P]
    lib.saber_hip_conv2d_chain_create3_pair.argtypes = [P, P, P, P, C.POINTER(P)]
    lib.saber_hip_conv2d_chain_run3.argtypes = [P, P, P, P, P, P, P]
    lib.saber_hip_conv2d_chain_set_tile.argtypes = [P, I]
    lib.saber_hip_conv2d_chain_get_tile.argtypes = [P]
    lib.saber_hip_conv2d_stage_create.argtypes = [C.POINTER(P), I, C.POINTER(P)]
    lib.saber_hip_conv2d_stage_destroy.argtypes = [P]
    lib.saber_hip_conv2d_stage_destroy.restype = None
    lib.saber_hip_conv2d_stage_run.argtypes = [P, P, P, C.POINTER(P), C.POINTER(P), P]
    lib.saber_hip_conv2d_stage_create_tail.argtypes = [C.POINTER(P), I, P, C.POINTER(P)]
    lib.saber_hip_conv2d_stage_run_tail.argtypes = [P, P, P, C.POINTER(P), C.POINTER(P), P, P]
    lib.saber_hip_conv2d_stage_create_head.argtypes = [C.POINTER(P), I, P, P, P, C.POINTER(P)]
    lib.saber_hip_conv2d_stage_run_head.argtypes = [P, P, P, C.POINTER(P), C.POINTER(P), P, P]
    lib.saber_hip_conv2d_stem_pair_create.argtypes = [P, P, P, C.POINTER(P)]
    lib.saber_hip_conv2d_stem_pair_destroy.argtypes = [P]
    lib.saber_hip_conv2d_stem_pair_destroy.restype = None
    lib.saber_hip_conv2d_stem_pair_run.argtypes = [P, P, P, P, P, P, P]
    lib.saber_hip_conv2d_sep_create.argtypes = [P, P, C.POINTER(P)]
    lib.saber_hip_conv2d_sep_run.argtypes = [P, P, P, P, P]
    lib.saber_hip_conv2d_sep_set_tile.argtypes = [P, I]
    lib.saber_hip_conv2d_sep_get_tile.argtypes = [P]
    lib.saber_hip_conv2d_sep_algo.argtypes = [P]
    lib.saber_hip_conv2d_sep_algo.restype = C.c_char_p
    lib.saber_hip_conv2d_sep_destroy.argtypes = [P]
    lib.saber_hip_conv2d_sep_destroy.restype = None
    lib.saber_hip_conv2d_ir_create.argtypes = [P, P, P, C.POINTER(P)]
    lib.saber_hip_conv2d_ir_run.argtypes = [P, P, P, P, P, P]
    lib.saber_hip_conv2d_ir_set_tile.argtypes = [P, I]
    lib.saber_hip_conv2d_ir_get_tile.argtypes = [P]
    lib.saber_hip_conv2d_ir_algo.argtypes = [P]
    lib.saber_hip_conv2d_ir_algo.restype = C.c_char_p
    lib.saber_hip_conv2d_ir_destroy.argtypes = [P]
    lib.saber_hip_conv2d_ir_destroy.restype = None
    lib.saber_hip_conv2d_set_global_pooling.argtypes = [P]
    lib.saber_hip_conv2d_run_gpool.argtypes = [P, P, P, P, P, P]
    lib.saber_hip_stage_create.argtypes = [C.POINTER(StagePhase), I, C.POINTER(P)]
    lib.saber_hip_stage_num_tensors.argtypes = [P]
    lib.saber_hip_stage_run.argtypes = [P, C.POINTER(P), I, P]
    lib.saber_hip_stage_status.argtypes = [P]
    lib.saber_hip_stage_trace.argtypes = [P, P, C.c_size_t]
    lib.saber_hip_stage_destroy.argtypes = [P]
    lib.saber_hip_stage_destroy.restype = None
    lib.saber_hip_fc_create.argtypes = [C.POINTER(FcDesc), C.POINTER(P)]
    lib.saber_hip_fc_set_weights.argtypes = [P, P, I, P, P, F, F]
    lib.saber_hip_fc_workspace_bytes.argtypes = [P]
    lib.saber_hip_fc_workspace_bytes.restype = Z
    lib.saber_hip_fc_run.argtypes = [P, P, P, P, P]
    lib.saber_hip_fc_destroy.argtypes = [P]
    lib.saber_hip_net_optimize.argtypes = [P, I]
    lib.saber_hip_net_stage_blocks.argtypes = [P, I]
    lib.saber_hip_net_stage_head.argtypes = [P, I]
    lib.saber_hip_net_status.argtypes = [P]
    lib.saber_hip_net_inject_coop_error.argtypes = [P]
    lib.saber_hip_net_coop_fallbacks.argtypes = [P]
    lib.saber_hip_coop_fallbacks_total.argtypes = []
    lib.saber_hip_net_time_op_in_pass.argtypes = [P, P, I, I, C.POINTER(C.c_float)]
    lib.saber_hip_net_get_choice.argtypes = [P, I]
    lib.saber_hip_net_set_choice.argtypes = [P, I, I]
    lib.saber_hip_fc_algo.argtypes = [P]
    lib.saber_hip_fc_algo.restype = C.c_char_p
    lib.saber_hip_fc_set_tile.argtypes = [P, I]
    lib.saber_hip_fc_destroy.restype = None
    lib.saber_hip_gemm_f32.argtypes = [I, I, I, I, I, F, P, P, F, P, P]
    lib.saber_hip_gemm_f32_release_plans.argtypes = []
    lib.saber_hip_gemm_f32_release_plans.restype = I
    lib.saber_hip_gemm_i8_create.argtypes = [I, I, I, I, I, I, P, C.POINTER(P)]
    lib.saber_hip_gemm_i8_workspace_bytes.argtypes = [P]
    lib.saber_hip_gemm_i8_workspace_bytes.restype = Z
    lib.saber_hip_gemm_i8_run.argtypes = [P, P, P, P, P]
    lib.saber_hip_gemm_i8_destroy.argtypes = [P]
    lib.saber_hip_gemm_i8_destroy.restype = None
    lib.saber_hip_quantize_nchw_to_nhwc.argtypes = [I, I, I, I, I, I, F, P, P, P]
    lib.saber_hip_dequantize_nhwc_to_nchw.argtypes = [I, I, I, I, I, F, P, P, P]
    lib.saber_hip_transpose_nchw_to_nhwc_f32.argtypes = [I, I, I, I, I, P, P, P]
    lib.saber_hip_transpose_nhwc_to_nchw_f32.argtypes = [I, I, I, I, I, P, P, P]
    lib.saber_hip_quantize_flat_s8.argtypes = [Z, F, P, P, P]
    lib.saber_hip_eltwise_sum_i8.argtypes = [Z, P, P, F, F, F, F, I, P, P]
    lib.saber_hip_eltwise_sum_f32.argtypes = [Z, P, P, F, F, I, P, P]
    lib.saber_hip_pool_out_dim.argtypes = [I, I, I, I, I]
    lib.saber_hip_pool_out_dim2.argtypes = [I, I, I, I, I, I]
    lib.saber_hip_pool2d_i8_nhwc.argtypes = [I] * 15 + [P, P, P]
    lib.saber_hip_pool2d_f32.argtypes = [I] * 14 + [P, P, P]
    lib.saber_hip_pool2d_f32_from_i8.argtypes = [I] * 14 + [F, P, P, P]
    lib.saber_hip_pool2d_f32_from_i8_q.argtypes = [I] * 14 + [F, P, P, F, P, P]
# ... 109 lines not shown
```

anakin_amd/saber.py:

```python
import ctypes as C

import numpy as np
import torch

from . import lib as L

_TORCH_DT = {L.F32: torch.float32, L.S8: torch.int8, L.U8: torch.uint8}


def _stream():
    return C.c_void_p(torch.cuda.current_stream().cuda_stream)


def _p(t):
    return None if t is None else C.c_void_p(t.data_ptr())


def _np_ptr(a):
    return None if a is None else a.ctypes.data_as(C.c_void_p)


def dtype_code(t):
    return {torch.float32: L.F32, torch.int8: L.S8, torch.uint8: L.U8}[t.dtype]

# ... 283 lines not shown
    def autotune(self, x, ya, yb, iters=5):
        L.check(L.load().saber_hip_conv2d_autotune_pair(self.h, _p(x), _p(ya), _p(yb), _stream(), iters))

    def __del__(self):
        try:
            if self.h:
                L.load().saber_hip_conv2d_destroy(self.h)
        except Exception:
            pass


ACTIVE_SIGMOID, ACTIVE_RELU, ACTIVE_TANH, ACTIVE_CLIPPED_RELU, ACTIVE_ELU, ACTIVE_STANH, ACTIVE_PRELU, ACTIVE_GELU, ACTIVE_SWISH = \
    1, 2, 3, 4, 5, 9, 10, 11, 12


def activation(active, x, y=None, negative_slope=0.0, coef=1.0):
    import torch
    if y is None:
        y = torch.empty_like(x)
    L.check(L.load().saber_hip_activation_f32(int(active), x.numel(), float(negative_slope), float(coef), _p(x), _p(y), _stream()))
    return y


def prelu(x, slope, channels, inner, channel_shared=False, y=None):
    import torch
    if y is None:
        y = torch.empty_like(x)
    L.check(L.load().saber_hip_prelu_f32(x.numel(), int(channels), int(inner), int(bool(channel_shared)), _p(slope), _p(x), _p(y), _stream()))
    return y


class SaberConvChain:

    def __init__(self, a, b, conv3x3=None, pair_b=None):
        self.a, self.b, self.c3, self.b2 = a, b, conv3x3, pair_b
        self.h = C.c_void_p()
        if pair_b is not None:
            L.check(L.load().saber_hip_conv2d_chain_create3_pair(conv3x3.h, a.h, b.h, pair_b.h, C.byref(self.h)))
        elif conv3x3 is None:
            L.check(L.load().saber_hip_conv2d_chain_create(a.h, b.h, C.byref(self.h)))
        else:
            L.check(L.load().saber_hip_conv2d_chain_create3(conv3x3.h, a.h, None if b is None else b.h, C.byref(self.h)))

    def dispatch(self, x, res, ya, yb=None, yc=None):
        L.check(L.load().saber_hip_conv2d_chain_run3(self.h, _p(x), _p(res), _p(ya), _p(yb), _p(yc), _stream()))
        return ya, yb

    def set_tile(self, tn):
        L.check(L.load().saber_hip_conv2d_chain_set_tile(self.h, tn))

    def tile(self):
        return L.load().saber_hip_conv2d_chain_get_tile(self.h)

    def __del__(self):
        try:
            if self.h:
                L.load().saber_hip_conv2d_chain_destroy(self.h)
        except Exception:
            pass


class SaberChainStage:

    def __init__(self, chains, tail=None, head=None):
        self.chains = list(chains)
        self.tail = tail
        self.head = head
        arr = (C.c_void_p * len(chains))(*[c.h for c in chains])
        self.h = C.c_void_p()
        if head is not None:
            L.check(L.load().saber_hip_conv2d_stage_create_head(arr, len(chains), tail.h if tail is not None else None, head[0].h, head[1].h,
                                                                C.byref(self.h)))
        elif tail is None:
            L.check(L.load().saber_hip_conv2d_stage_create(arr, len(chains), C.byref(self.h)))
        else:
            L.check(L.load().saber_hip_conv2d_stage_create_tail(arr, len(chains), tail.h, C.byref(self.h)))

    def dispatch(self, x, res, y1s, y2s, y_tail=None):
        n = len(self.chains)
# ... 613 lines not shown
        self.set_choices(ch)

    def tails(self):
        ch = self.choices()
        return [(i, n) for i, n, on in self.stages() if on and (ch[i] >> 31) & 1]

    def select_tails(self, on):
        ch = self.choices()
        for i, _, sel in self.stages():
            if sel:
                v = ((ch[i] | (1 << 31)) if on else (ch[i] & ~(1 << 31))) & 0xffffffff
                ch[i] = v - (1 << 32) if v >> 31 else v
        self.set_choices(ch)

    def heads(self):
        lib = L.load()
        ch = self.choices()
        out = []
        for i, _, on in self.stages():
            p = int(lib.saber_hip_net_stage_head(self.h, i))
            if on and p >= 0 and (ch[p] >> 29) & 1:
                out.append((p, i))
        return out

    def select_heads(self, on):
        lib = L.load()
        ch = self.choices()
        for i, _, sel in self.stages():
            p = int(lib.saber_hip_net_stage_head(self.h, i))
            if sel and p >= 0:
                ch[p] = (ch[p] | (1 << 29)) if on else (ch[p] & ~(1 << 29))
        self.set_choices(ch)

    def time_ops(self, iters=20):
        out = (C.c_float * self.num_ops())()
        L.check(L.load().saber_hip_net_time_ops(self.h, _stream(), iters, out))
        return list(out)

    def time_op_in_pass(self, index, iters=20):
        out = C.c_float()
        L.check(L.load().saber_hip_net_time_op_in_pass(self.h, _stream(), int(index), int(iters), C.byref(out)))
        return float(out.value)

    def time_pass(self, iters=20):
        out = (C.c_float * self.num_ops())()
        L.check(L.load().saber_hip_net_time_pass(self.h, _stream(), iters, out))
        return list(out)

    def op_work(self, index):
        b, f = C.c_double(), C.c_double()
        L.check(L.load().saber_hip_net_op_work(self.h, int(index), C.byref(b), C.byref(f)))
        return b.value, f.value

    def arena_bytes(self):
        return L.load().saber_hip_net_arena_bytes(self.h)

    def compact(self, keep=()):
        ids = (C.c_int * max(1, len(keep)))(*[self.tensors[k][0] for k in keep])
        L.check(L.load().saber_hip_net_compact_arena(self.h, ids, len(keep)))
        return self.arena_bytes()

    def compacted(self):
        return bool(L.load().saber_hip_net_arena_compacted(self.h))

    def tensor_of_ptr(self, t):
        return int(L.load().saber_hip_net_tensor_of_ptr(self.h, t.data_ptr()))
# ... 44 lines not shown
```

anakin_amd/workloads.py:

```python
import numpy as np

F32, S8, U8 = 0, 1, 2


def resnet_spec(depth=50):
    return _bottleneck_spec({50: [3, 4, 6, 3], 101: [3, 4, 23, 3]}[depth], 64, 4, 1, False)


def resnext_spec():
    return _bottleneck_spec([3, 4, 6, 3], 128, 2, 32, True)


def _bottleneck_spec(blocks, width, expand, group, stride_3x3):
    L = []
    L.append(dict(kind="conv", name="conv1", src="data", cin=3, cout=64, k=7, stride=2, pad=3, relu=True))
    L.append(dict(kind="pool", name="pool1", src="conv1", win=3, stride=2, pad=0, type=0))
    prev, cin, hw = "pool1", 64, 56
    for si, nb in enumerate(blocks):
        mid = width << si
        cout = mid * expand
        for bi in range(nb):
            stride = 2 if (bi == 0 and si > 0) else 1
            tag = "res%d%s" % (si + 2, chr(ord("a") + bi) if nb <= 6 else ("a" if bi == 0 else "b%d" % bi))
            if bi == 0:
# ... 241 lines not shown
                if l["relu"]:
                    y = torch.relu(y)
            elif kd == "pool":
                y = Fn.max_pool2d(t[l["src"]], l["win"], l["stride"], l["pad"], ceil_mode=not l.get("floor", False))
            elif kd == "eltwise":
                y = t[l["a"]] + t[l["b"]]
                if l["relu"]:
                    y = torch.relu(y)
            elif kd == "gpool":
                y = t[l["src"]].mean((2, 3), keepdim=True)
            elif kd == "fc":
                w, b = model["params"][l["name"]]
                y = Fn.linear(t[l["src"]].flatten(1), torch.from_numpy(w), torch.from_numpy(b))
                if l.get("relu"):
                    y = torch.relu(y)
            elif kd == "softmax":
                y = torch.softmax(t[l["src"]], 1)
            elif kd == "concat":
                t[l["name"]] = torch.cat([t[s] for s in l["srcs"]], 1)
                scales[l["name"]] = max(scales[s] for s in l["srcs"])
                for s in l["srcs"]:
                    scales[s] = scales[l["name"]]
                continue
            t[l["name"]] = y
            scales[l["name"]] = max(float(y.abs().max()), 1e-6) / 127.0
    return scales


def _out_hw(h, k, s, p):
    return (h + 2 * p - k) // s + 1


def build_int8_net(model, scales, batch, hw=224, fuse=True, chain=2, stage=True, stem_pair=True, head_pair=False, shared_device=False,
                   fc_softmax=True, absorb_pool=True, separable=False, inverted=False, fire=False, before_finalize=None, **legacy):
    from . import lib as L
    from . import saber as S
    legacy.pop("cxx_optimize", None)
    chain = 2 if chain is None else chain
    if legacy:
        raise TypeError("build_int8_net: %s belong to the Python fuser, which is test infrastructure now (tests/py_fuser.py)" % sorted(legacy))
    net = S.Net()
    B = batch
    net.add_tensor("data", (B, 3, hw, hw), F32)
    shape = {"data": (hw, 3)}
    dtype = {"data": F32}
    scales = dict(scales)
    for l in model["spec"]:
        kd, nm = l["kind"], l["name"]
        if kd == "conv":
            hin, cin = shape[l["src"]]
            ho = _out_hw(hin, l["k"], l["stride"], l["pad"])
            w, b = model["params"][nm]
            odt = l.get("odt", U8 if l["relu"] else S8)
            p = S.ConvParam(w, b, l.get("group", 1), (l["pad"],) * 2, (l["stride"],) * 2, (1, 1), l["relu"])
            shape[nm], dtype[nm] = (ho, l["cout"]), odt
            conv = S.SaberConv2D(True).init((B, cin, hin, hin), p, dtype[l["src"]], odt, scales[l["src"]], scales[nm],
                                            in_layout=L.NCHW if dtype[l["src"]] == F32 else L.NHWC)
            net.add_tensor(nm, (B, ho, ho, l["cout"]), odt)
            net.add_conv(conv, l["src"], nm)
        elif kd == "pool":
            hin, c = shape[l["src"]]
            ho = S.pool_out_dim(hin, l["pad"], l["win"], l["stride"], l.get("floor", False))
            shape[nm], dtype[nm] = (ho, c), dtype[l["src"]]
            scales[nm] = scales[l["src"]]
            net.add_tensor(nm, (B, ho, ho, c), dtype[nm])
            net.add_pool_i8(B, hin, hin, c, ho, ho, (l["win"],) * 2, (l["stride"],) * 2, (l["pad"],) * 2, l["type"],
                            dtype[l["src"]], dtype[nm], l["src"], nm)
# ... 19 lines not shown
        elif kd == "gpool":
            hin, c = shape[l["src"]]
            net.add_tensor(nm, (B, c, 1, 1), F32)
            net.add_pool_f32_from_i8(B, hin, hin, c, 1, 1, (hin, hin), (hin, hin), (0, 0), 1, dtype[l["src"]],
                                     scales[l["src"]], l["src"], nm)
            shape[nm], dtype[nm] = (1, c), F32
        elif kd == "fc":
            w, b = model["params"][nm]
            fc = S.SaberFc(True).init(B, l["cout"], l["cin"], w, b, dtype.get(l["src"], F32), scales[l["src"]])
            net.add_tensor(nm, (B, l["cout"]), F32)
            net.add_fc(fc, l["src"], nm)
        elif kd == "softmax":
            classes = next(e.get("cout", shape.get(l["src"], (0, 0))[1]) for e in model["spec"] if e["name"] == l["src"])
            net.add_tensor(nm, (B, classes), F32)
            net.add_softmax(B, classes, l["src"], nm)
    net.unfused_ops = net.num_ops()
    if shared_device:
        net.optimize(2048)
        stage = False
    net.removed = net.absorbed = net.gpooled = net.stem_paired = net.chained = net.fc_softmaxed = net.separated = net.inverted = net.fired = 0
    if fuse:
        net.removed = net.optimize(15)
    if fire:
        net.fired = net.optimize(65536)
    if inverted:
        net.inverted = net.optimize(32768)
    if separable:
        net.separated = net.optimize(16384)
    if fuse:
        net.absorbed = net.optimize(64) if absorb_pool else 0
        net.gpooled = net.optimize(128) if absorb_pool else 0
        net.stem_paired = net.optimize(512) if stem_pair else 0
        net.chained = net.optimize(16 | (32 if int(chain) >= 2 else 0) | (256 if int(chain) >= 2 and stage else 0) |
                                   (1024 if int(chain) >= 2 and head_pair else 0)) if chain else 0
        net.fc_softmaxed = net.optimize(4096) if fc_softmax else 0
    if before_finalize is not None:
        before_finalize(net)
    net.finalize()
    return net


def build_fp32_net(model, batch, hw=224, pair_siblings=True, fuse_pool=True, shared_device=False, reproducible=False, fuse_stem=True,
                   fc_softmax=True):
    from . import lib as L
    from . import saber as S
    net = S.Net()
    B = batch
    net.add_tensor("data", (B, 3, hw, hw), F32)
    spec = model["spec"]
    shape, alias = {}, {}
    fused_away = set()
    done_convs = set()
    produced = []
    l0, l1 = spec[0], (spec[1] if len(spec) > 1 else None)
    if fuse_stem and l0["kind"] == "conv" and l0["src"] == "data" and l1 is not None and l1["kind"] == "pool" and l1["src"] == l0["name"] \
            and l1["type"] == 0 and l0["relu"] and sum(1 for e in spec for k in ("src", "a", "b") if e.get(k) == l0["name"]) == 1:
        w0, b0 = model["params"][l0["name"]]
        p0 = S.ConvParam(w0, b0, 1, (l0["pad"],) * 2, (l0["stride"],) * 2, (1, 1), True)
        cp0 = S.SaberConv2DPooling(int8=False).init((B, 3, hw, hw), p0, l1["type"], (l1["win"],) * 2, (l1["stride"],) * 2, (l1["pad"],) * 2,
                                                     F32, F32, floor_mode=l1.get("floor", False), in_layout=L.NCHW)
        if cp0.fused and cp0.algo().startswith("stem7x7s2_maxpool3x3s2_f32"):
            po = cp0.out_hw[0]
            net.add_tensor(l1["name"], (B, po, po, l0["cout"]), F32)
            shape[l1["name"]] = (po, l0["cout"])
            net.add_conv(cp0.conv, "data", l1["name"])
            net.keep.append(cp0)
            produced.append((net.num_ops() - 1, l1["name"]))
# ... 144 lines not shown
```

include/saber_hip.h:

```cpp
#ifndef SABER_HIP_H
#define SABER_HIP_H

#include <stddef.h>
#include <stdint.h>

#ifdef __cplusplus
extern "C" {
#endif

typedef void* saber_hip_stream_t;

typedef enum {
    SABER_HIP_OK = 0,
    SABER_HIP_INVALID_VALUE = -2,
    SABER_HIP_UNIMPL = -3,
    SABER_HIP_OUT_OF_MEM = -4,
    SABER_HIP_RUNTIME_ERROR = -5
} saber_hip_status;

typedef enum { SABER_HIP_F32 = 0, SABER_HIP_S8 = 1, SABER_HIP_U8 = 2, SABER_HIP_S32 = 3 } saber_hip_dtype;
typedef enum { SABER_HIP_NHWC = 0, SABER_HIP_NCHW = 1 } saber_hip_layout;
typedef enum { SABER_HIP_ACT_NONE = 0, SABER_HIP_ACT_RELU = 1 } saber_hip_act;
typedef enum { SABER_HIP_POOL_MAX = 0, SABER_HIP_POOL_AVG_INCL = 1, SABER_HIP_POOL_AVG_EXCL = 2 } saber_hip_pool_type;

// ... 30 lines not shown
typedef struct saber_hip_conv saber_hip_conv_t;

int saber_hip_conv2d_create(const saber_hip_conv_desc* desc, saber_hip_conv_t** out);
int saber_hip_conv2d_set_weights(saber_hip_conv_t* op, const void* w, int w_dtype, const float* w_scale,
                                 const float* bias, float in_scale, float out_scale);
size_t saber_hip_conv2d_workspace_bytes(const saber_hip_conv_t* op);
void saber_hip_conv2d_out_shape(const saber_hip_conv_t* op, int* oh, int* ow);
int saber_hip_conv2d_run(saber_hip_conv_t* op, const void* x, void* y, const void* res, void* workspace,
                         saber_hip_stream_t stream);
void saber_hip_conv2d_destroy(saber_hip_conv_t* op);
int saber_hip_conv2d_set_pooling(saber_hip_conv_t* op, int pool_type, int kh, int kw, int stride_h, int stride_w,
                                 int pad_h, int pad_w, int floor_mode);
int saber_hip_conv2d_get_quantized_weights(const saber_hip_conv_t* op, int8_t* wq_oihw, float* w_scale);
const char* saber_hip_conv2d_algo(const saber_hip_conv_t* op);
int saber_hip_conv2d_set_tile(saber_hip_conv_t* op, int tile);
int saber_hip_conv2d_get_tile(const saber_hip_conv_t* op);
int saber_hip_conv2d_autotune(saber_hip_conv_t* op, const void* x, void* y, const void* res, void* workspace,
                              saber_hip_stream_t stream, int iters);

int saber_hip_conv2d_set_global_pooling(saber_hip_conv_t* op);
int saber_hip_conv2d_run_gpool(saber_hip_conv_t* op, const void* x, void* y, const void* res, void* y_pool,
                               saber_hip_stream_t stream);

int saber_hip_conv2d_create_pair(const saber_hip_conv_t* a, const saber_hip_conv_t* b, saber_hip_conv_t** out);
int saber_hip_conv2d_run_pair(saber_hip_conv_t* pair, const void* x, void* y_a, void* y_b, saber_hip_stream_t stream);
int saber_hip_conv2d_autotune_pair(saber_hip_conv_t* pair, const void* x, void* y_a, void* y_b,
                                   saber_hip_stream_t stream, int iters);

typedef struct saber_hip_chain saber_hip_chain_t;
int saber_hip_conv2d_chain_create(saber_hip_conv_t* a, saber_hip_conv_t* b, saber_hip_chain_t** out);
int saber_hip_conv2d_chain_create3(saber_hip_conv_t* conv3x3, saber_hip_conv_t* a, saber_hip_conv_t* b, saber_hip_chain_t** out);
int saber_hip_conv2d_chain_create3_pair(saber_hip_conv_t* conv3x3, saber_hip_conv_t* a, saber_hip_conv_t* pair_a, saber_hip_conv_t* pair_b,
                                        saber_hip_chain_t** out);
void saber_hip_conv2d_chain_destroy(saber_hip_chain_t* chain);
int saber_hip_conv2d_chain_run(saber_hip_chain_t* chain, const void* x, const void* res, void* y_a, void* y_b,
                               saber_hip_stream_t stream);
int saber_hip_conv2d_chain_run3(saber_hip_chain_t* chain, const void* x, const void* res, void* y_a, void* y_b, void* y_c,
                                saber_hip_stream_t stream);
int saber_hip_conv2d_chain_set_tile(saber_hip_chain_t* chain, int tn);
int saber_hip_conv2d_chain_get_tile(const saber_hip_chain_t* chain);

typedef struct saber_hip_chain_stage saber_hip_chain_stage_t;
int saber_hip_conv2d_stage_create(saber_hip_chain_t* const* chains, int n, saber_hip_chain_stage_t** out);
void saber_hip_conv2d_stage_destroy(saber_hip_chain_stage_t* stage);
int saber_hip_conv2d_stage_run(saber_hip_chain_stage_t* stage, const void* x, const void* res, void* const* y1, void* const* y2,
                               saber_hip_stream_t stream);
int saber_hip_conv2d_stage_create_tail(saber_hip_chain_t* const* chains, int n, saber_hip_chain_t* tail, saber_hip_chain_stage_t** out);
int saber_hip_conv2d_stage_run_tail(saber_hip_chain_stage_t* stage, const void* x, const void* res, void* const* y1, void* const* y2,
                                    void* y_tail, saber_hip_stream_t stream);

int saber_hip_conv2d_stage_create_head(saber_hip_chain_t* const* chains, int n, saber_hip_chain_t* tail, const saber_hip_conv_t* head_a,
                                       const saber_hip_conv_t* head_b, saber_hip_chain_stage_t** out);
int saber_hip_conv2d_stage_run_head(saber_hip_chain_stage_t* stage, const void* x_head, void* y_head_b, void* const* y1, void* const* y2,
                                    void* y_tail, saber_hip_stream_t stream);

typedef struct saber_hip_stem_pair saber_hip_stem_pair_t;
int saber_hip_conv2d_stem_pair_create(saber_hip_conv_t* stem, const saber_hip_conv_t* a, const saber_hip_conv_t* b, saber_hip_stem_pair_t** out);
void saber_hip_conv2d_stem_pair_destroy(saber_hip_stem_pair_t* sp);
int saber_hip_conv2d_stem_pair_run(saber_hip_stem_pair_t* sp, const void* x, void* y_pool, void* y_a, void* y_b, void* workspace,
                                   saber_hip_stream_t stream);

typedef struct saber_hip_sep saber_hip_sep_t;
int saber_hip_conv2d_sep_create(saber_hip_conv_t* dw, saber_hip_conv_t* pw, saber_hip_sep_t** out);
int saber_hip_conv2d_sep_run(saber_hip_sep_t* sep, const void* x, void* y_dw , void* y_pw, saber_hip_stream_t stream);
int saber_hip_conv2d_sep_set_tile(saber_hip_sep_t* sep, int code);
int saber_hip_conv2d_sep_get_tile(const saber_hip_sep_t* sep);
// ... 109 lines not shown
int saber_hip_net_create(saber_hip_net_t** out);
int saber_hip_net_add_tensor(saber_hip_net_t* net, size_t bytes);
int saber_hip_net_add_conv(saber_hip_net_t* net, saber_hip_conv_t* op, int in_id, int out_id, int res_id);
int saber_hip_net_add_conv_pair(saber_hip_net_t* net, saber_hip_conv_t* pair, int in_id, int out_a_id, int out_b_id);
int saber_hip_net_add_fc(saber_hip_net_t* net, saber_hip_fc_t* op, int in_id, int out_id);
int saber_hip_net_add_quantize(saber_hip_net_t* net, int n, int c, int h, int w, int c_pad, int out_dtype,
                               float scale, int in_id, int out_id);
int saber_hip_net_add_dequantize(saber_hip_net_t* net, int n, int c, int h, int w, int in_dtype, float scale,
                                 int in_id, int out_id);
int saber_hip_net_add_transpose_in_f32(saber_hip_net_t* net, int n, int c, int h, int w, int c_pad, int in_id,
                                       int out_id);
int saber_hip_net_add_eltwise_i8(saber_hip_net_t* net, size_t count, float scale_a, float scale_b,
                                 float coeff_a, float coeff_b, int relu, int a_id, int b_id, int out_id);
int saber_hip_net_add_eltwise_f32(saber_hip_net_t* net, size_t count, float coeff_a, float coeff_b, int relu,
                                  int a_id, int b_id, int out_id);
int saber_hip_net_add_pool_i8(saber_hip_net_t* net, int n, int h, int w, int c, int oh, int ow, int kh, int kw,
                              int stride_h, int stride_w, int pad_h, int pad_w, int pool_type, int in_dtype,
                              int out_dtype, int in_id, int out_id);
int saber_hip_net_add_pool_f32(saber_hip_net_t* net, int n, int h, int w, int c, int oh, int ow, int kh, int kw,
                               int stride_h, int stride_w, int pad_h, int pad_w, int pool_type, int layout,
                               int in_id, int out_id);
int saber_hip_net_add_pool_f32_from_i8(saber_hip_net_t* net, int n, int h, int w, int c, int oh, int ow, int kh,
                                       int kw, int stride_h, int stride_w, int pad_h, int pad_w, int pool_type,
                                       int in_dtype, float scale, int in_id, int out_id);
int saber_hip_net_add_pool_f32_from_i8_q(saber_hip_net_t* net, int n, int h, int w, int c, int oh, int ow, int kh, int kw,
                                         int stride_h, int stride_w, int pad_h, int pad_w, int pool_type, int in_dtype,
                                         float scale, int in_id, int out_id, float q_scale, int q_out_id);
int saber_hip_net_add_fc_q(saber_hip_net_t* net, saber_hip_fc_t* op, int in_q_id, int out_id);
#define SABER_HIP_NET_SHARED_DEVICE 2048
#define SABER_HIP_NET_REPRODUCIBLE_FP32 8192
#define SABER_HIP_NET_SEPARABLE 16384
#define SABER_HIP_NET_INVERTED_RESIDUAL 32768
#define SABER_HIP_NET_FIRE 65536
int saber_hip_net_optimize(saber_hip_net_t* net, int flags);
int saber_hip_net_coop_fallbacks(const saber_hip_net_t* net);
int saber_hip_coop_fallbacks_total(void);
int saber_hip_net_status(saber_hip_net_t* net);
int saber_hip_net_inject_coop_error(saber_hip_net_t* net);
int saber_hip_net_stage_blocks(const saber_hip_net_t* net, int index);
int saber_hip_net_stage_head(const saber_hip_net_t* net, int index);
int saber_hip_net_num_launches(const saber_hip_net_t* net);
int saber_hip_net_tensor_unwritten(const saber_hip_net_t* net, int id);
int saber_hip_net_add_softmax(saber_hip_net_t* net, int rows, int cols, int in_id, int out_id);
int saber_hip_net_set_lane(saber_hip_net_t* net, int op_index, int lane);
int saber_hip_net_finalize(saber_hip_net_t* net);
void* saber_hip_net_tensor_ptr(saber_hip_net_t* net, int id);
size_t saber_hip_net_arena_bytes(const saber_hip_net_t* net);
int saber_hip_net_compact_arena(saber_hip_net_t* net, const int* keep, int n_keep);
int saber_hip_net_arena_compacted(const saber_hip_net_t* net);
int saber_hip_net_num_ops(const saber_hip_net_t* net);
int saber_hip_net_run(saber_hip_net_t* net, saber_hip_stream_t stream);
int saber_hip_net_run_op(saber_hip_net_t* net, int index, saber_hip_stream_t stream);
int saber_hip_net_capture(saber_hip_net_t* net, saber_hip_stream_t stream);
int saber_hip_net_replay(saber_hip_net_t* net, saber_hip_stream_t stream);
int saber_hip_net_time_ops(saber_hip_net_t* net, saber_hip_stream_t stream, int iters, float* out_us);
int saber_hip_net_time_pass(saber_hip_net_t* net, saber_hip_stream_t stream, int iters, float* out_us);
int saber_hip_net_time_op_in_pass(saber_hip_net_t* net, saber_hip_stream_t stream, int index, int iters, float* out_us);
int saber_hip_net_op_work(const saber_hip_net_t* net, int index, double* bytes, double* flops);
const char* saber_hip_net_op_name(const saber_hip_net_t* net, int index);
int saber_hip_net_get_choice(saber_hip_net_t* net, int index);
int saber_hip_net_set_choice(saber_hip_net_t* net, int index, int choice);
int saber_hip_net_autotune(saber_hip_net_t* net, saber_hip_stream_t stream, int iters);
void saber_hip_net_destroy(saber_hip_net_t* net);
int saber_hip_net_add_relu_f32(saber_hip_net_t* net, size_t count, int in_id, int out_id);
int saber_hip_net_add_activation_f32(saber_hip_net_t* net, int active, size_t count, float negative_slope, float coef, int in_id,
                                     int out_id);
int saber_hip_net_add_concat(saber_hip_net_t* net, size_t pixels, int n_inputs, const int* in_ids, const int* channels,
                             const float* mult, int dtype, int out_id);
int saber_hip_net_add_deconv(saber_hip_net_t* net, saber_hip_deconv_t* op, int in_id, int out_id);
int saber_hip_net_bind_tensor(saber_hip_net_t* net, int id, void* ptr);
int saber_hip_net_num_tensors(const saber_hip_net_t* net);
size_t saber_hip_net_tensor_bytes(const saber_hip_net_t* net, int id);

// ... 12 lines not shown
```

integration/mi355x/framework/mi355x_net_planner.h:

```cpp
#ifndef ANAKIN_FRAMEWORK_CORE_NET_MI355X_NET_PLANNER_H
#define ANAKIN_FRAMEWORK_CORE_NET_MI355X_NET_PLANNER_H

namespace anakin {

template <typename Ttype, Precision Ptype, OpRunType RunType>
struct MI355XPlanner {
    static bool run(Net<Ttype, Ptype, RunType>&) { return false; }
    static void prepare(Net<Ttype, Ptype, RunType>&) {}
};

#ifdef USE_MI355X_PLACE
template <Precision Ptype, OpRunType RunType>
struct MI355XPlanner<saber::MI355X, Ptype, RunType> {
    typedef Net<saber::MI355X, Ptype, RunType> net_t;
    typedef saber::TargetWrapper<saber::MI355X> API;

    static bool env_on(const char* name, bool dflt) {
        const char* e = std::getenv(name);
        return e ? e[0] != '0' : dflt;
    }
    static std::vector<int> dims(Tensor4dPtr<saber::MI355X> t) {
        saber::Shape s = t->valid_shape();
        std::vector<int> v;
        for (int i = 0; i < s.dims(); ++i) v.push_back(s[i]);
// ... 26 lines not shown
            plan.in_t.push_back((void*)t);
            plan.in_ptr.push_back(t->data());
            plan.in_shape.push_back(dims(t));
        }
        bool ok = plan.captured_ops > 0;
        for (auto& t : net.get_out_list()) {
            const int id = saber_hip_net_tensor_of_ptr(n, t->data());
            ok = ok && id >= 0 && saber_hip_net_bind_tensor(n, id, t->mutable_data()) == SABER_HIP_OK;
            plan.out_t.push_back((void*)t);
            plan.out_ptr.push_back(t->data());
        }
        plan.stream = (void*)net._exec_funcs[0].ctx_p->get_compute_stream();
        {
            const char* own = std::getenv("SABER_MI355X_NET_PLAN_STREAM");
            if (own && std::string(own) == "own") plan.want_own_stream = true;
            if (plan.want_own_stream) plan.shared_device = true;
            if (plan.want_own_stream && !plan.own_stream) {
                API::stream_t s;
                API::event_t e;
                API::create_stream_with_flag(&s, 1);
                API::owner_syncs_stream(s);
                API::create_event(&e, false);
                plan.own_stream = (void*)s;
                plan.own_event = (void*)e;
            }
        }
        void* const ctx_stream = plan.stream;
        if (plan.own_stream) plan.stream = plan.own_stream;
        plan.ctx_stream = ctx_stream;
        const bool stage = !plan.shared_device && env_on("SABER_MI355X_NET_STAGE", true);
        const bool stem_pair = env_on("SABER_MI355X_NET_STEM_PAIR", true);
        const bool head_pair = env_on("SABER_MI355X_NET_HEAD_PAIR", false);
        const bool fc_softmax = env_on("SABER_MI355X_NET_FC_SOFTMAX", true);
        if (ok) ok = saber_hip_net_optimize(n, 255 | (stage ? 256 : 0) | (stem_pair ? 512 : 0) | (head_pair ? 1024 : 0) | (fc_softmax ? 4096 : 0) |
                                               (plan.shared_device ? SABER_HIP_NET_SHARED_DEVICE : 0) |
                                               (MI355XNetPlanDefaults::reproducible_fp32() ? SABER_HIP_NET_REPRODUCIBLE_FP32 : 0)) >= 0;
        if (ok) ok = saber_hip_net_finalize(n) == SABER_HIP_OK;
        if (ok && plan.builds == 0 && env_on("SABER_MI355X_NET_PLAN_TUNE", true))
            ok = saber_hip_net_autotune(n, plan.stream, 9) == SABER_HIP_OK;
        if (ok && env_on("SABER_MI355X_NET_PLAN_COMPACT", plan.shared_device)) {
            plan.arena_bytes_full = saber_hip_net_arena_bytes(n);
            ok = saber_hip_net_compact_arena(n, nullptr, 0) == SABER_HIP_OK;
        }
        plan.arena_bytes = saber_hip_net_arena_bytes(n);
        if (!plan.arena_bytes_full) plan.arena_bytes_full = plan.arena_bytes;
        if (ok) ok = choose_launch_form(n, plan);
        if (!ok) {
            plan.why = saber_hip_last_error();
            LOG(WARNING) << "MI355X net plan: " << plan.why << " - Net::prediction keeps the operator loop";
            saber_hip_net_destroy(n);
            return;
        }
        plan.net = n;
        plan.launches = saber_hip_net_num_launches(n);
        ++plan.builds;
        LOG(INFO) << "MI355X net plan: " << net._exec_funcs.size() << " executors -> " << plan.captured_ops << " captured ops -> "
                  << plan.launches << " launches per prediction (" << (plan.use_graph ? "hipGraph replay" : "eager") << "), arena "
                  << (plan.arena_bytes >> 20) << " MiB (every edge materialised: " << (plan.arena_bytes_full >> 20) << " MiB)";
    }

    static bool choose_launch_form(saber_hip_net_t* n, MI355XNetPlan& plan) {
        const char* force = std::getenv("SABER_MI355X_NET_PLAN_GRAPH");
        if (force && force[0] == '0') { plan.use_graph = false; return true; }
        if (saber_hip_net_capture(n, plan.stream) != SABER_HIP_OK) { plan.use_graph = false; return true; }
        if (force) { plan.use_graph = true; return true; }
        API::event_t e0, e1;
        API::create_event(&e0, true);
// ... 75 lines not shown
```

Baseline: 39860.

## Fuse the stage-transition 1x1 conv pair into the following C=128 chain kernel

Adds a chain-head kernel form that computes the 256->512 shortcut and 256->128 1x1 conv pair inside the 8-wave C=128 conv3x3 chain kernel, so both no longer run as a separate launch. The change packs the head weights into their own stream, extends the net optimizer, lane/reader tracking and autotune choice bits, and turns the feature on by default through a new optimize flag. The aim is to remove a kernel launch and a round trip of the intermediate tensors through memory at the stage boundary. In exchange the chain kernel carries more work and register pressure, and the dependency bookkeeping gets more complex.

```diff
diff --git a/anakin_amd/build.py b/anakin_amd/build.py
--- a/anakin_amd/build.py
+++ b/anakin_amd/build.py
@@ -5,7 +5,7 @@
 HERE = os.path.dirname(os.path.abspath(__file__))
 CSRC = os.path.join(HERE, "csrc")
 LIB = os.path.join(HERE, "libsaber_mi355x.so")
-SOURCES = ["conv_igemm.hip", "elementwise.hip", "fc_small.hip", "conv1x1_chain.hip", "conv_chain_coop.hip", "conv_stage_coop.hip", "stage_xcd.hip", "conv1x1_gpool.hip", "conv3x3_b3h.hip", "conv1x1_pw.hip", "conv1x1_pwk.hip", "conv_stem_f32.hip", "fc_f32_splitk.hip", "conv_dw3x3.hip", "conv_group3x3.hip", "conv_sep.hip", "conv_ir.hip", "conv_fire.hip", "deconv.hip"] + \
+SOURCES = ["conv_igemm.hip", "elementwise.hip", "fc_small.hip", "conv1x1_chain.hip", "conv_chain_head.hip", "conv_chain_coop.hip", "conv_stage_coop.hip", "stage_xcd.hip", "conv1x1_gpool.hip", "conv3x3_b3h.hip", "conv1x1_pw.hip", "conv1x1_pwk.hip", "conv_stem_f32.hip", "fc_f32_splitk.hip", "conv_dw3x3.hip", "conv_group3x3.hip", "conv_sep.hip", "conv_ir.hip", "conv_fire.hip", "deconv.hip"] + \
     ["api_%s.hip" % n for n in ("conv", "select", "autotune", "ops", "chain", "sep", "ir", "fire", "deconv", "stage", "net", "net_optimize", "net_autotune", "capture", "gemm", "streams")] + \
     ["igemm_m%d_e%d.hip" % me for me in [(0, 0), (0, 1), (0, 2), (0, 3), (0, 4), (1, 0), (1, 1), (1, 2), (1, 3), (2, 3), (3, 3)]] + \
     ["igemm_dma_m%d_e%d.hip" % me for me in [(0, 0), (0, 1), (0, 2), (0, 3), (0, 4), (2, 3)]] + \
diff --git a/anakin_amd/csrc/api_chain.hip b/anakin_amd/csrc/api_chain.hip
--- a/anakin_amd/csrc/api_chain.hip
+++ b/anakin_amd/csrc/api_chain.hip
@@ -1,14 +1,14 @@
 #include "api_internal.h"
 
-enum : unsigned { CK_1X1 = 1, CK_3X3 = 2, CK_HEAD = 4, CK_PAIR = 8, CK_LED = CK_3X3 | CK_HEAD, CK_ANY = 15 };
+enum : unsigned { CK_1X1 = 1, CK_3X3 = 2, CK_HEAD = 4, CK_PAIR = 8, CK_LED = CK_3X3 | CK_HEAD, CK_ANY = 15, CK_PHEAD = 16 };
 static unsigned chain_kind(const saber_hip_chain* ch) { return !ch->c3 ? CK_1X1 : (ch->b2 ? CK_PAIR : (ch->b ? CK_3X3 : CK_HEAD)); }
 static const struct { int c1; unsigned kinds; ChainForm f; } chain_forms[] = {
     {64, CK_ANY,            {4, 4, 4, 1, 1, CS_BASE, false}},
     {64, CK_ANY,            {2, 2, 4, 1, 1, CS_BASE, false}},
     {128, CK_1X1 | CK_LED,  {2, 2, 4, 1, 1, CS_BASE, false}},
     {128, CK_1X1 | CK_LED,  {1, 1, 4, 1, 1, CS_BASE, false}},
-    {128, CK_1X1 | CK_LED,  {6, 2, 8, 1, 1, CS_W8, false}},
-    {128, CK_1X1 | CK_LED,  {5, 1, 8, 1, 1, CS_W8, false}},
+    {128, CK_1X1 | CK_LED | CK_PHEAD,  {6, 2, 8, 1, 1, CS_W8, false}},
+    {128, CK_1X1 | CK_LED | CK_PHEAD,  {5, 1, 8, 1, 1, CS_W8, false}},
     {256, CK_1X1 | CK_LED,  {1, 1, 4, 1, 1, CS_BASE, false}},
     {256, CK_1X1,           {9, 1, 4, 2, 1, CS_SPLIT, false}},
     {256, CK_1X1,           {11, 1, 8, 2, 1, CS_SPLIT8, false}},
@@ -33,6 +33,12 @@
 bool chain_form_valid(const saber_hip_chain* ch, int code) {
     const ChainForm f = chain_form(ch, code);
     return f.code && ch->d_stream[f.stream].p && (f.coop != 4 || ch->stage1);
+}
+bool chain_form_has_head(const saber_hip_chain* ch, int code) {
+    if (!ch || !ch->head_a || !ch->d_head_stream.p) return false;
+    for (const auto& r : chain_forms)
+        if (r.c1 == ch->c1 && (r.kinds & chain_kind(ch)) && (r.kinds & CK_PHEAD) && r.f.code == code) return chain_form_valid(ch, code);
+    return false;
 }
 std::string chain_form_name(const saber_hip_chain* ch) {
     const ChainForm& f = ch->form;
@@ -570,12 +576,8 @@
                                saber_hip_stream_t stream) {
     return saber_hip_conv2d_chain_run3(ch, x, res, y_a, y_b, nullptr, stream);
 }
-int saber_hip_conv2d_chain_run3(saber_hip_chain_t* ch, const void* x, const void* res, void* y_a, void* y_b, void* y_c,
-                                saber_hip_stream_t stream) {
-    if (g_capture) return capture_unsupported("saber_hip_conv2d_chain_run (saber_hip_net_optimize forms chains itself)");
-    if (!ch || !x || !res || !y_a || (ch->b && !y_b) || (ch->b2 && !y_c)) return fail(SABER_HIP_INVALID_VALUE, "null argument");
+static int chain_fill_args(const saber_hip_chain* ch, const void* x, const void* res, void* y_a, void* y_b, void* y_c, ChainKArgs& k) {
     const saber_hip_conv *a = ch->a, *b = ch->b;
-    ChainKArgs k;
     std::memset(&k, 0, sizeof k);
     k.x = x; k.res = res;
     const ChainForm f = ch->form;
@@ -613,6 +615,16 @@
         k.H0 = ch->c3->d.h; k.W0 = ch->c3->d.w;
         if (a->d.res_stride > 1) { k.res_sub = a->d.res_stride; k.res_H = a->d.res_h; k.res_W = a->d.res_w; }
     }
+    return SABER_HIP_OK;
+}
+int saber_hip_conv2d_chain_run3(saber_hip_chain_t* ch, const void* x, const void* res, void* y_a, void* y_b, void* y_c,
+                                saber_hip_stream_t stream) {
+    if (g_capture) return capture_unsupported("saber_hip_conv2d_chain_run (saber_hip_net_optimize forms chains itself)");
+    if (!ch || !x || !res || !y_a || (ch->b && !y_b) || (ch->b2 && !y_c)) return fail(SABER_HIP_INVALID_VALUE, "null argument");
+    ChainKArgs k;
+    const int rk = chain_fill_args(ch, x, res, y_a, y_b, y_c, k);
+    if (rk) return rk;
+    const ChainForm f = ch->form;
     if (f.coop == 4) {
         const int rc = stage_run(ch->stage1, x, res, &y_a, &y_b, (hipStream_t)stream);
         if (rc != SABER_HIP_OK) ch->form = chain_form_plain(ch);
@@ -632,3 +644,70 @@
     HIP_TRY(launch_conv1x1_chain(k, ch->c1, ch->k1, ch->k2, f.rows, f.waves, f.split, ch->c3 ? 1 : 0, (hipStream_t)stream));
     return SABER_HIP_OK;
 }
+
+void pack_chain_head_stream(const int8_t* wa, const int8_t* wb, std::vector<uint8_t>& out) {
+    const int C0 = 256;
+    for (int w = 0; w < 8; ++w) {
+        for (int ks = 0; ks < 4; ++ks)
+            for (int mf = 0; mf < 4; ++mf) pack_frag1(wa, C0, w * 64, 4, mf, ks, out);
+        for (int ks = 0; ks < 4; ++ks) pack_frag1(wb, C0, w * 16, 1, 0, ks, out);
+    }
+}
+int saber_hip_conv2d_chain_create3_head(const saber_hip_conv_t* pair_a, const saber_hip_conv_t* pair_b, saber_hip_conv_t* conv3x3, saber_hip_conv_t* a,
+                                        saber_hip_conv_t* b, saber_hip_chain_t** out) {
+    if (!pair_a || !pair_b || !conv3x3 || !a || !b || !out) return fail(SABER_HIP_INVALID_VALUE, "null argument");
+    for (const saber_hip_conv* o : {pair_a, pair_b}) {
+        const saber_hip_conv_desc& d = o->d;
+        if (!o->is_i8 || !o->weights_set || o->algo != ALGO_IGEMM_I8 || o->epi != EPI_I8_CONV || o->pair_k2 || o->pool_fused || o->pool2 || o->gpool ||
+            o->pre_quant || o->pre_pad || d.kh != 1 || d.kw != 1 || d.stride_h != 1 || d.stride_w != 1 || d.pad_h != 0 || d.pad_w != 0 || d.group != 1 ||
+            o->c_eff != d.c || d.act_negative_slope != 0.f || d.in_layout != SABER_HIP_NHWC || d.out_layout != SABER_HIP_NHWC ||
+            d.res_mode != SABER_HIP_RES_NONE || (d.out_dtype != SABER_HIP_S8 && d.out_dtype != SABER_HIP_U8) || d.c != 256 ||
+            (int)o->wq_oihw.size() != d.k * 256)
+            return fail(SABER_HIP_UNIMPL, "chain head: the pair must be two plain 1x1 / stride 1 / pad 0 INT8 NHWC convs over 256 channels with weights set");
+    }
+    const saber_hip_conv_desc &pa = pair_a->d, &pb = pair_b->d, &d3 = conv3x3->d, &da = a->d;
+    if (pa.k != 512 || pb.k != 128 || da.c != 128 || d3.stride_h != 1 || d3.stride_w != 1 || da.res_stride > 1)
+        return fail(SABER_HIP_UNIMPL, "chain head: 256 -> 512 | 128 in front of a stride-1 conv3x3 + chain at C = 128 only");
+    if (pa.n != d3.n || pa.h != d3.h || pa.w != d3.w || pb.n != d3.n || pb.h != d3.h || pb.w != d3.w || pair_a->x_dtype != pair_b->x_dtype ||
+        pa.out_dtype != SABER_HIP_S8 || (pb.out_dtype == SABER_HIP_U8) != (conv3x3->x_dtype == DT_U8))
+        return fail(SABER_HIP_UNIMPL, "chain head: the pair's outputs must be the chain's shortcut (s8) and its 3x3 conv's input (its dtype), on the chain's pixels, one input tensor");
+    saber_hip_chain* ch = nullptr;
+    const int rc = chain_build(conv3x3, a, b, &ch);
+    if (rc) return rc;
+    std::vector<uint8_t> hs, p1, p2, prm(512 * 16, 0);
+    pack_chain_head_stream(pair_a->wq_oihw.data(), pair_b->wq_oihw.data(), hs);
+    pack_chain_params(pair_a, 384, p1);
+    pack_chain_params(pair_b, 96, p2);
+    std::memcpy(prm.data(), p1.data(), p1.size());
+    std::memcpy(prm.data() + p1.size(), p2.data(), p2.size());
+    hipError_t e = ch->d_head_stream.upload(hs);
+    if (e == hipSuccess) e = ch->d_head_prm.upload(prm);
+    if (e != hipSuccess) {
+        delete ch;
+        return hip_fail(e, "chain head: device copies");
+    }
+    ch->head_a = pair_a; ch->head_b = pair_b;
+    ch->head_in_u8 = pair_a->x_dtype == DT_U8;
+    ch->head_relu_a = pa.act == SABER_HIP_ACT_RELU; ch->head_relu_b = pb.act == SABER_HIP_ACT_RELU;
+    if (!chain_form_has_head(ch, 6) && !chain_form_has_head(ch, 5)) {
+        delete ch;
+        return fail(SABER_HIP_UNIMPL, "chain head: no kernel form of this chain takes a head");
+    }
+    *out = ch;
+    return SABER_HIP_OK;
+}
+int saber_hip_conv2d_chain_run3_head(saber_hip_chain_t* ch, const void* x_pair, void* y_a, void* y_b, saber_hip_stream_t stream) {
+    if (g_capture) return capture_unsupported("saber_hip_conv2d_chain_run3_head (saber_hip_net_optimize forms chains itself)");
+    if (!ch || !x_pair || !y_a || !y_b) return fail(SABER_HIP_INVALID_VALUE, "null argument");
+    if (!ch->head_a) return fail(SABER_HIP_INVALID_VALUE, "chain: created without a head");
+    if (!chain_form_has_head(ch, ch->form.code)) return fail(SABER_HIP_INVALID_VALUE, "chain: the selected form runs no head (8 waves: set_tile 6 | 5)");
+    saber_mi355x::ChainHeadKArgs k;
+    std::memset(&k, 0, sizeof k);
+    const int rk = chain_fill_args(ch, x_pair, nullptr, y_a, y_b, nullptr, k.c);
+    if (rk) return rk;
+    k.hstream = ch->d_head_stream.p; k.hprm = ch->d_head_prm.p;
+    k.hin_u8 = ch->head_in_u8; k.hrelu_a = ch->head_relu_a; k.hrelu_b = ch->head_relu_b;
+    HIP_TRY(saber_mi355x::launch_conv_chain_head_c128(k, ch->form.rows, (hipStream_t)stream));
+    return SABER_HIP_OK;
+}
+int saber_hip_conv2d_chain_has_head(const saber_hip_chain_t* ch, int tn) { return chain_form_has_head(ch, tn ? tn : (ch ? ch->form.code : 0)) ? 1 : 0; }
diff --git a/anakin_amd/csrc/api_internal.h b/anakin_amd/csrc/api_internal.h
--- a/anakin_amd/csrc/api_internal.h
+++ b/anakin_amd/csrc/api_internal.h
@@ -203,6 +203,10 @@
     int c1 = 0, k1 = 0, k2 = 0;
     float scale_conv = 1.f;
     std::vector<int8_t> tail_w3, tail_wa;
+    const saber_hip_conv* head_a = nullptr;
+    const saber_hip_conv* head_b = nullptr;
+    DevBuf<uint8_t> d_head_stream, d_head_prm;
+    bool head_in_u8 = false, head_relu_a = false, head_relu_b = false;
     ChainForm form;
     DevBuf<uint8_t> d_stream[CS_COUNT];
     DevBuf<uint8_t> d_prm0, d_prm1, d_prm2;
@@ -381,6 +385,8 @@
     int chain3_res = -1, chain3_y1 = -1, chain3_y2 = -1;
     int chain3_y3 = -1;
     bool led_on = false;
+    bool pair_head_on = false;
+    int pair_head_of = -1;
     saber_hip_chain_stage* stage = nullptr;
     int stage_n = 0;
     bool stage_on = false;
@@ -505,6 +511,8 @@
 void net_drop_graph(saber_hip_net* net);
 void net_set_chain_mode(saber_hip_net* net, int ia, int mode);
 int net_chain_mode(const saber_hip_net* net, int ia);
+void net_set_pair_head(saber_hip_net* net, int i3, bool on);
+bool net_pair_head_effective(const saber_hip_net* net, int i3);
 void net_set_stage(saber_hip_net* net, int i0, bool on);
 void net_set_head(saber_hip_net* net, int i0, bool on);
 void net_set_tail(saber_hip_net* net, int i0, bool on);
@@ -513,6 +521,7 @@
 ChainForm chain_form_default(const saber_hip_chain* ch);
 ChainForm chain_form_plain(const saber_hip_chain* ch);
 std::string chain_form_name(const saber_hip_chain* ch);
+bool chain_form_has_head(const saber_hip_chain* ch, int code);
 void for_each_chain_candidate(const saber_hip_chain* ch, bool shared_device, const std::function<void(const ChainForm&)>& fn);
 bool conv_sep_ok(const saber_hip_conv* dw, const saber_hip_conv* pw, std::string* why);
 bool sep_form_valid(const saber_hip_sep* sp, int code);
diff --git a/anakin_amd/csrc/api_net.hip b/anakin_amd/csrc/api_net.hip
--- a/anakin_amd/csrc/api_net.hip
+++ b/anakin_amd/csrc/api_net.hip
@@ -37,6 +37,8 @@
         }
         case LAUNCH_STEM_PAIR: return saber_hip_conv2d_stem_pair_run(o.stem_pair, T(o.in), nullptr, T(o.stem_y1), T(o.stem_y2), ws, s);
         case LAUNCH_CHAIN3: {
+            const int io = (int)(&o - net->ops.data());
+            if (io > 0 && net->ops[io - 1].absorbed_by == io) return saber_hip_conv2d_chain_run3_head(o.chain3, T(net->ops[io - 1].in), T(o.chain3_y1), T(o.chain3_y2), s);
             const int rc = saber_hip_conv2d_chain_run3(o.chain3, T(o.in), T(o.chain3_res), T(o.chain3_y1), T(o.chain3_y2), T(o.chain3_y3), s);
             if (rc == SABER_HIP_RUNTIME_ERROR) {
                 ++net->coop_fallbacks;
@@ -334,6 +336,7 @@
         if (o.stage) span(i, 3 * o.stage_n + (o.stage->tail ? 2 : 0));
         if (o.stage && o.stage->head_a && i > 0) span(i - 1, 2);
         if (o.chain3) span(i, 3);
+        if (o.chain3 && o.chain3->head_a && i > 0) span(i - 1, 2);
         if (o.chain) span(i, 2);
         if (o.stem_pair) span(i, 2);
         if (o.sep) span(i, 2);
@@ -412,6 +415,7 @@
 const char* saber_hip_net_op_name(const saber_hip_net_t* net, int i) {
     return (i >= 0 && i < (int)net->ops.size()) ? net->ops[i].name.c_str() : "";
 }
+static int net_front_cover(const NetOp& o) { return o.pair_head_of >= 0 ? o.pair_head_of : o.head_of; }
 static int net_prepare_lanes(saber_hip_net* net) {
     if (net->lanes_ready) return SABER_HIP_OK;
     const int nops = (int)net->ops.size();
@@ -437,7 +441,8 @@
             rd[t].clear();
             w[t] = i;
         }
-        op_for_each_input(o, [&](int t) { rd[t].push_back(i); });
+        const int fc = net_front_cover(o);
+        op_for_each_input(o, [&](int t) { rd[t].push_back(i); if (fc >= 0) rd[t].push_back(fc); });
     }
     if (net->has_side) {
         HIP_TRY(hipStreamCreateWithFlags(&net->side, hipStreamNonBlocking));
@@ -491,7 +496,8 @@
         if (o.lane) side_dirty = true;
         net->writer[o.out] = (int)i;
         if (o.out2 >= 0) net->writer[o.out2] = (int)i;
-        op_for_each_input(o, [&](int t) { readers[t].push_back((int)i); });
+        const int fc = net_front_cover(o);
+        op_for_each_input(o, [&](int t) { readers[t].push_back((int)i); if (fc >= 0) readers[t].push_back(fc); });
     }
     if (side_dirty) {
         HIP_TRY(hipEventRecord(net->ev_join, net->side));
@@ -568,6 +574,8 @@
         conv_work(o.conv, *bytes, *flops);
         for (int j = index + 1; j < (int)net->ops.size(); ++j)
             if (net->ops[j].absorbed_by == index && net->ops[j].conv) conv_work(net->ops[j].conv, *bytes, *flops);
+        if (o.launch == LAUNCH_CHAIN3 && index > 0 && net->ops[index - 1].absorbed_by == index && net->ops[index - 1].conv)
+            conv_work(net->ops[index - 1].conv, *bytes, *flops);
         return SABER_HIP_OK;
     case OP_CONV_PAIR:
         if (!o.skip) conv_work(o.conv, *bytes, *flops);
@@ -685,6 +693,7 @@
         if (o.out == id && (o.launch == LAUNCH_IR || (o.skip && by == LAUNCH_IR && (int)(&o - net->ops.data()) == o.absorbed_by + 1))) return 1;
         if (o.out == id && o.kind == OP_CONV && (o.launch == LAUNCH_FIRE || (o.skip && by == LAUNCH_FIRE))) return 1;
         if (o.launch == LAUNCH_STAGE && o.head_on && o.chain3_res == id) return 1;
+        if (o.launch == LAUNCH_CHAIN3 && net_pair_head_effective(net, (int)(&o - net->ops.data())) && (o.chain3_res == id || o.in == id)) return 1;
         if (o.chain3 && o.stage_y1_private && o.chain3_y1 == id && (o.launch == LAUNCH_STAGE || (o.skip && by == LAUNCH_STAGE))) return 1;
     }
     return 0;
diff --git a/anakin_amd/csrc/api_net_autotune.hip b/anakin_amd/csrc/api_net_autotune.hip
--- a/anakin_amd/csrc/api_net_autotune.hip
+++ b/anakin_amd/csrc/api_net_autotune.hip
@@ -22,7 +22,18 @@
     if (o.stage && o.stage_on) choice |= 1 << 30;
     if (o.stage && o.stage_on && o.tail_on) choice |= (int)0x80000000u;
     if (o.head_of >= 0 && net->ops[o.head_of].stage_on && net->ops[o.head_of].head_on) choice |= 1 << 29;
+    if (o.pair_head_of >= 0 && net_pair_head_effective(net, o.pair_head_of)) choice |= 1 << 28;
     return choice;
+}
+int saber_hip_net_chain_head(const saber_hip_net_t* net, int index) {
+    if (!net || index < 1 || index >= (int)net->ops.size() || !net->ops[index].chain3) return -1;
+    return net->ops[index - 1].pair_head_of == index ? index - 1 : -1;
+}
+int saber_hip_net_set_chain_head(saber_hip_net_t* net, int index, int on) {
+    if (saber_hip_net_chain_head(net, index) < 0) return fail(SABER_HIP_INVALID_VALUE, "op `index` leads no chain with a pair head");
+    net_set_pair_head(net, index, on != 0);
+    net_drop_graph(net);
+    return SABER_HIP_OK;
 }
 int saber_hip_net_stage_blocks(const saber_hip_net_t* net, int index) {
     if (!net || index < 0 || index >= (int)net->ops.size()) return 0;
@@ -85,6 +96,7 @@
     if (o.stage) net_set_stage(net, index, stage_on);
     if (o.stage) net_set_tail(net, index, tail_on);
     if (o.head_of >= 0) net_set_head(net, o.head_of, (chain_bits & 32) && !net->shared_device);
+    if (o.pair_head_of >= 0) net_set_pair_head(net, o.pair_head_of, (chain_bits & 16) != 0);
     if (sep_bits) net_set_sep(net, index, tn);
     if (ir_bits) net_set_ir(net, index, ir_tn);
     if (fire_bits) net_set_fire(net, index, ir_tn);
@@ -241,6 +253,7 @@
         auto timed = [&](float* t) { return time_enqueued(s, run_all, 20, t); };
         float best = 0.f;
         int best_mode = 0, best_tn = 0;
+        if (H) net_set_pair_head(net, ia - 1, false);
         net_set_chain_mode(net, ia, 0);
         int rc = timed(&best);
         if (rc) return rc;
@@ -258,6 +271,30 @@
         }
         if (best_mode) (void)saber_hip_conv2d_chain_set_tile(best_mode == 2 ? H->chain3 : A.chain, best_tn);
         net_set_chain_mode(net, ia, best_mode);
+        if (H && saber_hip_net_chain_head(net, ia - 1) >= 0) {
+            auto run_pair_too = [&]() -> int { return net_launch(net, net->ops[ia - 2], s) | run_all(); };
+            float base = 0.f, best_h = 0.f;
+            int head_tn = 0;
+            rc = time_enqueued(s, run_pair_too, 20, &base);
+            if (rc) return rc;
+            log_cand(A.conv, "pair + " + (best_mode ? (best_mode == 2 ? H->name : A.name).substr(5) : std::string("separate")), base);
+            const int keep_tn = H->chain3->form.code;
+            for_each_chain_candidate(H->chain3, net->shared_device, [&](const ChainForm& f) {
+                float ms = -1.f;
+                if (!chain_form_has_head(H->chain3, f.code) || saber_hip_conv2d_chain_set_tile(H->chain3, f.code) != SABER_HIP_OK) return;
+                net_set_chain_mode(net, ia, 2);
+                net_set_pair_head(net, ia - 1, true);
+                const int rt = time_enqueued(s, run_pair_too, 20, &ms);
+                log_cand(A.conv, H->name.substr(5), ms);
+                if (rt == SABER_HIP_OK && (!head_tn || ms < best_h)) { best_h = ms; head_tn = f.code; }
+            });
+            const bool keep = head_tn && best_h < base * 0.99f;
+            (void)saber_hip_conv2d_chain_set_tile(H->chain3, keep ? head_tn : keep_tn);
+            net_set_chain_mode(net, ia, keep ? 2 : best_mode);
+            net_set_pair_head(net, ia - 1, keep);
+            rc = net_launch(net, net->ops[ia - 2], s);
+            if (rc) return rc;
+        }
         rc = run_all();
         if (rc) return rc;
     }
@@ -270,7 +307,7 @@
         hipStream_t s = (hipStream_t)stream;
         auto run_all = [&]() -> int {
             int rc = 0;
-            for (int k = first - (has_head ? 1 : 0); k <= last; ++k) rc |= net_launch(net, net->ops[k], s);
+            for (int k = first - (has_head || saber_hip_net_chain_head(net, first) >= 0 ? 1 : 0); k <= last; ++k) rc |= net_launch(net, net->ops[k], s);
             return rc;
         };
         auto timed = [&](float* t) { return time_enqueued(s, run_all, 20, t); };
diff --git a/anakin_amd/csrc/api_net_optimize.hip b/anakin_amd/csrc/api_net_optimize.hip
--- a/anakin_amd/csrc/api_net_optimize.hip
+++ b/anakin_amd/csrc/api_net_optimize.hip
@@ -41,6 +41,7 @@
             o.launch = LAUNCH_CHAIN3;
             absorb(i + 1, i, IN_CHAIN);
             if (o.chain3->b || o.chain3->b2) absorb(i + 2, i, IN_CHAIN);
+            if (net_pair_head_effective(net, i)) absorb(i - 1, i, IN_CHAIN);
         } else if (o.chain && o.chain_on) {
             o.launch = LAUNCH_CHAIN;
             absorb(i + 1, i, IN_CHAIN);
@@ -75,7 +76,7 @@
             case LAUNCH_NONE: o.name = covered[kept ? IN_STAGE : in[i]]; break;
             case LAUNCH_OWN: o.name = "conv:" + own + o.res_note; break;
             case LAUNCH_CHAIN: o.name = "conv:" + chain_form_name(o.chain); break;
-            case LAUNCH_CHAIN3: o.name = "conv:" + chain_form_name(o.chain3); break;
+            case LAUNCH_CHAIN3: o.name = std::string(net_pair_head_effective(net, i) ? "conv:[pair1x1]+" : "conv:") + chain_form_name(o.chain3); break;
             case LAUNCH_SEP: o.name = std::string("conv:") + saber_hip_conv2d_sep_algo(o.sep); break;
             case LAUNCH_IR: o.name = std::string("conv:") + saber_hip_conv2d_ir_algo(o.ir); break;
             case LAUNCH_FIRE: o.name = std::string("conv:") + saber_hip_conv2d_fire_algo(o.fire); break;
@@ -100,6 +101,17 @@
 int net_chain_mode(const saber_hip_net* net, int ia) {
     const NetOp& A = net->ops[ia];
     return (ia > 0 && net->ops[ia - 1].chain3 && net->ops[ia - 1].led_on) ? 2 : (A.chain_on ? 1 : 0);
+}
+bool net_pair_head_effective(const saber_hip_net* net, int i3) {
+    if (i3 < 1 || i3 >= (int)net->ops.size()) return false;
+    const NetOp& H = net->ops[i3];
+    return H.chain3 && H.led_on && H.pair_head_on && net->ops[i3 - 1].pair_head_of == i3 && !(H.stage && H.stage_on) &&
+           chain_form_has_head(H.chain3, H.chain3->form.code);
+}
+void net_set_pair_head(saber_hip_net* net, int i3, bool on) {
+    if (i3 < 1 || i3 >= (int)net->ops.size() || net->ops[i3 - 1].pair_head_of != i3) return;
+    net->ops[i3].pair_head_on = on;
+    net_resolve(net);
 }
 void net_set_tail(saber_hip_net* net, int i0, bool on) {
     NetOp& H0 = net->ops[i0];
@@ -513,9 +525,21 @@
                 continue;
             if (readers(Hd.out) != 1) continue;
             saber_hip_chain* ch = nullptr;
-            if (saber_hip_conv2d_chain_create3(Hd.conv, A.conv, B.conv, &ch) != SABER_HIP_OK) continue;
+            bool headed = false;
+            if ((flags & SABER_HIP_NET_CHAIN_HEAD) && i >= 1) {
+                const NetOp& P = ops[i - 1];
+                const int t_res = A.in2, t_x = Hd.in;
+                if (P.kind == OP_CONV_PAIR && !P.skip && !P.lane && P.conv && P.conv->pair_src_a && P.conv->pair_src_b && P.pair_head_of < 0 && P.head_of < 0 &&
+                    t_res != t_x && ((P.out == t_res && P.out2 == t_x) || (P.out == t_x && P.out2 == t_res)) && readers(t_res) == 1 && readers(t_x) == 1) {
+                    const bool fwd = P.out == t_res;
+                    headed = saber_hip_conv2d_chain_create3_head(fwd ? P.conv->pair_src_a : P.conv->pair_src_b, fwd ? P.conv->pair_src_b : P.conv->pair_src_a,
+                                                                 Hd.conv, A.conv, B.conv, &ch) == SABER_HIP_OK;
+                }
+            }
+            if (!headed && saber_hip_conv2d_chain_create3(Hd.conv, A.conv, B.conv, &ch) != SABER_HIP_OK) continue;
             net->owned_chains.push_back(ch);
             Hd.chain3 = ch;
+            if (headed) ops[i - 1].pair_head_of = (int)i;
             Hd.chain3_res = A.in2; Hd.chain3_y1 = A.out; Hd.chain3_y2 = B.out;
             const bool was = A.chain_on;
             net_set_chain_mode(net, (int)i + 1, ch->c1 <= 128 ? 2 : (was ? 1 : 0));
@@ -530,7 +554,8 @@
             if (readers(Hd.out) != 1) continue;
             saber_hip_chain* ch = nullptr;
             NetOp* P = (flags & 1024) && i + 2 < ops.size() ? &ops[i + 2] : nullptr;
-            if (P && (P->kind != OP_CONV_PAIR || P->lane || P->skip || P->in != A.out || !P->conv || !P->conv->pair_src_a || !P->conv->pair_src_b)) P = nullptr;
+            if (P && (P->kind != OP_CONV_PAIR || P->lane || P->skip || P->pair_head_of >= 0 || P->in != A.out ||
+                      !P->conv || !P->conv->pair_src_a || !P->conv->pair_src_b)) P = nullptr;
             if (P) {
                 if (readers(A.out) != 1 || saber_hip_conv2d_chain_create3_pair(Hd.conv, A.conv, const_cast<saber_hip_conv*>(P->conv->pair_src_a),
                                                                    const_cast<saber_hip_conv*>(P->conv->pair_src_b), &ch) != SABER_HIP_OK)
diff --git a/anakin_amd/csrc/conv_chain_head.hip b/anakin_amd/csrc/conv_chain_head.hip
--- /dev/null
+++ b/anakin_amd/csrc/conv_chain_head.hip
@@ -0,0 +1,303 @@
+#include "epilogue_pack.h"
+
+namespace saber_mi355x {
+
+template <int TN>
+__global__ __launch_bounds__(512) void conv_chain_head_c128_kernel(const ChainHeadKArgs h) {
+    constexpr int NW = 8, R = 8;
+    constexpr int KSH = 4;
+    constexpr int KS1 = 2, KS2 = 8;
+    constexpr int K1 = 512, C1 = 128, K2 = 128;
+    constexpr int NPX = 16 * TN;
+    constexpr int TA = 16, TB = KSH, TH = TA + TB;
+    constexpr int T0 = 9 * KS1, T1 = KS1 * 4, T2 = KS2;
+    constexpr int TOT = TH + T0 + T1 + T2;
+    constexpr int CPR = K1 / 16, CH1 = C1 / 16, PCH = CH1 + 1;
+    constexpr int HW = 18, HP = (TN + 2) * HW;
+    constexpr int NF = (HP + 15) / 16;
+    constexpr int HCH = (HP * PCH + 63) / 64 * 64;
+    constexpr int XP = 17, XCH = (HP * XP + 63) / 64 * 64;
+    constexpr int P0C = 128, P1C = 384, P2C = 128, PHC = 512;
+    static_assert(T1 % R == 0 && T2 % R == 0 && TA % R == 0, "ring depth");
+
+    __shared__ v4i tile[NPX * CPR];
+    __shared__ v4i prm1[P1C];
+    __shared__ v4i prm2[P2C];
+    __shared__ v4i halo[HCH];
+    __shared__ v4i mid[NPX * PCH];
+    __shared__ v4i prm0[P0C];
+    __shared__ v4i xin[XCH];
+    __shared__ v4i prmh[PHC];
+    const ChainKArgs& a = h.c;
+    SABER_TL_DECL;
+    SABER_TL(0);
+    const int tid = threadIdx.x, lane = tid & 63;
+    const int wave = __builtin_amdgcn_readfirstlane(tid >> 6);
+    const int frow = lane & 15, fq = lane >> 4;
+    int n, y0, x0;
+    {
+        const int t = blockIdx.x;
+        n = a.mg_tpi ? (int)__umulhi((unsigned)t, a.mg_tpi) : t;
+        const int rem = t - n * a.tiles_per_img;
+        const int ty = a.mg_tiles_x ? (int)__umulhi((unsigned)rem, a.mg_tiles_x) : rem;
+        y0 = ty * TN;
+        x0 = (rem - ty * a.tiles_x) * 16;
+    }
+    auto pix = [&](int px, bool& ok) -> int {
+        int y = y0 + (px >> 4), x = x0 + (px & 15);
+        ok = y < a.H && x < a.W;
+        y = y < a.H ? y : a.H - 1;
+        x = x < a.W ? x : a.W - 1;
+        return (n * a.H + y) * a.W + x;
+    };
+    auto in_image = [&](int hp) -> bool {
+        const int hy = hp / HW, hx = hp - hy * HW;
+        return hp < HP && (unsigned)(y0 - 1 + hy) < (unsigned)a.H && (unsigned)(x0 - 1 + hx) < (unsigned)a.W;
+    };
+
+    {
+        const char* xg = (const char*)a.x;
+        for (int i = wave; i < XCH / 64; i += NW) {
+            const int L = i * 64 + lane;
+            const int hp = L / XP, cc = L - hp * XP;
+            const int hy = hp / HW, hx = hp - hy * HW;
+            const bool in = cc < 16 && in_image(hp);
+            const char* src = in ? xg + ((size_t)((n * a.H + (y0 - 1 + hy)) * a.W + (x0 - 1 + hx)) * 256 + cc * 16) : (const char*)a.zero;
+            lds_dma16(src, xin + i * 64);
+        }
+        for (int i = wave; i < PHC / 64; i += NW) lds_dma16((const v4i*)h.hprm + i * 64 + lane, prmh + i * 64);
+        for (int i = wave; i < P0C / 64; i += NW) lds_dma16((const v4i*)a.prm0 + i * 64 + lane, prm0 + i * 64);
+        for (int i = wave; i < P1C / 64; i += NW) lds_dma16((const v4i*)a.prm1 + i * 64 + lane, prm1 + i * 64);
+        for (int i = wave; i < P2C / 64; i += NW) lds_dma16((const v4i*)a.prm2 + i * 64 + lane, prm2 + i * 64);
+    }
+    asm volatile("" ::: "memory");
+
+    const v4i* hs = (const v4i*)h.hstream + (size_t)wave * (TH * 64) + lane;
+    const v4i* ws = (const v4i*)a.wstream + (size_t)wave * ((T0 + T1 + T2) * 64) + lane;
+    auto step = [&](int g) -> v4i { return g < TH ? hs[g * 64] : ws[(g - TH) * 64]; };
+    v4i ring[R];
+#pragma unroll
+    for (int r = 0; r < R; ++r) ring[r] = step(r);
+
+    asm volatile("s_waitcnt vmcnt(%0)" ::"n"(R) : "memory");
+    __builtin_amdgcn_s_barrier();
+    SABER_TL(6);
+    const int xmh = h.hin_u8 ? (int)0x80808080u : 0;
+
+    {
+        v4i bxa[KSH][TN];
+#pragma unroll
+        for (int j = 0; j < TN; ++j)
+#pragma unroll
+            for (int ks = 0; ks < KSH; ++ks) {
+                v4i b = xin[((j + 1) * HW + frow + 1) * XP + ks * 4 + fq];
+                b.x ^= xmh; b.y ^= xmh; b.z ^= xmh; b.w ^= xmh;
+                bxa[ks][j] = b;
+            }
+        const int cg = wave * 64 + fq * 16;
+        const v4i* pp = prmh + (cg / 4) * 3;
+        v4i acc[4][TN];
+#pragma unroll
+        for (int mf = 0; mf < 4; ++mf)
+#pragma unroll
+            for (int j = 0; j < TN; ++j) acc[mf][j] = pp[mf * 3 + 2];
+#pragma unroll
+        for (int s = 0; s < TA; ++s) {
+            const int ks = s / 4, mf = s % 4;
+#pragma unroll
+            for (int j = 0; j < TN; ++j) acc[mf][j] = mma_step(ring[s % R], bxa[ks][j], acc[mf][j]);
+            ring[s % R] = step(s + R);
+        }
+        const float loa = h.hrelu_a ? 0.f : -3.0e38f;
+#pragma unroll
+        for (int j = 0; j < TN; ++j) {
+            v4i o;
+            o.x = (int)chain_out_pack(acc[0][j], v4i{0, 0, 0, 0}, __builtin_bit_cast(v4f, pp[1]), __builtin_bit_cast(v4f, pp[0]), loa, 128.f, 0x80808080u);
+            o.y = (int)chain_out_pack(acc[1][j], v4i{0, 0, 0, 0}, __builtin_bit_cast(v4f, pp[4]), __builtin_bit_cast(v4f, pp[3]), loa, 128.f, 0x80808080u);
+            o.z = (int)chain_out_pack(acc[2][j], v4i{0, 0, 0, 0}, __builtin_bit_cast(v4f, pp[7]), __builtin_bit_cast(v4f, pp[6]), loa, 128.f, 0x80808080u);
+            o.w = (int)chain_out_pack(acc[3][j], v4i{0, 0, 0, 0}, __builtin_bit_cast(v4f, pp[10]), __builtin_bit_cast(v4f, pp[9]), loa, 128.f, 0x80808080u);
+            tile[(j * 16 + frow) * CPR + ((cg / 16) ^ frow)] = o;
+        }
+    }
+    SABER_TL(7);
+    {
+        const int c0 = wave * 16 + fq * 4;
+        const v4i* pp = prmh + P1C + (c0 / 4) * 3;
+        v4i acc[NF];
+        int xo[NF];
+#pragma unroll
+        for (int f = 0; f < NF; ++f) {
+            acc[f] = pp[2];
+            const int hp = f * 16 + frow;
+            xo[f] = (hp < HP ? hp : HP - 1) * XP + fq;
+        }
+#pragma unroll
+        for (int s = 0; s < TB; ++s) {
+#pragma unroll
+            for (int f = 0; f < NF; ++f) {
+                v4i b = xin[xo[f] + s * 4];
+                b.x ^= xmh; b.y ^= xmh; b.z ^= xmh; b.w ^= xmh;
+                acc[f] = mma_step(ring[(TA + s) % R], b, acc[f]);
+            }
+            ring[(TA + s) % R] = step(TA + s + R);
+        }
+        const float lob = h.hrelu_b ? 0.f : -3.0e38f;
+        const float offb = a.in0_u8 ? 0.f : 128.f;
+        const unsigned xob = a.in0_u8 ? 0u : 0x80808080u;
+#pragma unroll
+        for (int f = 0; f < NF; ++f) {
+            const int hp = f * 16 + frow;
+            const unsigned o = chain_out_pack(acc[f], v4i{0, 0, 0, 0}, __builtin_bit_cast(v4f, pp[1]), __builtin_bit_cast(v4f, pp[0]), lob, offb, xob);
+            if (hp < HP) *(unsigned*)((char*)halo + hp * (PCH * 16) + c0) = in_image(hp) ? o : 0u;
+        }
+    }
+    SABER_TL(8);
+    asm volatile("s_waitcnt lgkmcnt(0)" ::: "memory");
+    __builtin_amdgcn_s_barrier();
+    SABER_TL(1);
+
+    constexpr int G0 = TH;
+    v4i bx[KS1][TN];
+    {
+        const int xm0 = a.in0_u8 ? (int)0x80808080u : 0;
+        const int c0 = wave * (C1 / NW) + fq * 4;
+        const v4i* pp = prm0 + (c0 / 4) * 3;
+        v4i acc[TN];
+#pragma unroll
+        for (int j = 0; j < TN; ++j) acc[j] = pp[2];
+        const v4i* hb = halo + frow * PCH + fq;
+#pragma unroll
+        for (int s = 0; s < T0; ++s) {
+            const int ks = s % KS1, tap = s / KS1;
+            const int dy = tap / 3, dx = tap % 3;
+#pragma unroll
+            for (int j = 0; j < TN; ++j) {
+                v4i b = hb[((j + dy) * HW + dx) * PCH + ks * 4];
+                b.x ^= xm0; b.y ^= xm0; b.z ^= xm0; b.w ^= xm0;
+                acc[j] = mma_step(ring[(G0 + s) % R], b, acc[j]);
+            }
+            ring[(G0 + s) % R] = step(G0 + s + R);
+        }
+        const float lo0 = a.relu0 ? 0.f : -3.0e38f;
+        const float off0 = a.in_u8 ? 0.f : 128.f;
+        const unsigned xo0 = a.in_u8 ? 0u : 0x80808080u;
+#pragma unroll
+        for (int j = 0; j < TN; ++j) {
+            const unsigned o = chain_out_pack(acc[j], v4i{0, 0, 0, 0}, __builtin_bit_cast(v4f, pp[1]), __builtin_bit_cast(v4f, pp[0]), lo0, off0, xo0);
+            *(unsigned*)((char*)mid + (j * 16 + frow) * (PCH * 16) + c0) = o;
+        }
+        asm volatile("s_waitcnt lgkmcnt(0)" ::: "memory");
+        __builtin_amdgcn_s_barrier();
+#pragma unroll
+        for (int j = 0; j < TN; ++j)
+#pragma unroll
+            for (int ks = 0; ks < KS1; ++ks) bx[ks][j] = mid[(j * 16 + frow) * PCH + ks * 4 + fq];
+    }
+    const int xmask = a.in_u8 ? (int)0x80808080u : 0;
+#pragma unroll
+    for (int ks = 0; ks < KS1; ++ks)
+#pragma unroll
+        for (int j = 0; j < TN; ++j) {
+            bx[ks][j].x ^= xmask; bx[ks][j].y ^= xmask; bx[ks][j].z ^= xmask; bx[ks][j].w ^= xmask;
+        }
+    const float lo_s8 = a.relu1 ? 0.f : -128.f;
+    const float res_lo = a.res_relu ? 0.f : -3.0e38f;
+
+    constexpr int G1S = TH + T0;
+    {
+        v4i acc[4][TN];
+        const int cg = wave * 64 + fq * 16;
+        const v4i* pp = prm1 + (cg / 4) * 3;
+#pragma unroll
+        for (int mf = 0; mf < 4; ++mf)
+#pragma unroll
+            for (int j = 0; j < TN; ++j) acc[mf][j] = pp[mf * 3 + 2];
+#pragma unroll
+        for (int s = 0; s < T1; ++s) {
+            const int ks = s / 4, mf = s % 4;
+#pragma unroll
+            for (int j = 0; j < TN; ++j) acc[mf][j] = mma_step(ring[(G1S + s) % R], bx[ks][j], acc[mf][j]);
+            ring[(G1S + s) % R] = step(G1S + s + R);
+        }
+        SABER_TL(2);
+        v4f sc[4], bi[4];
+#pragma unroll
+        for (int mf = 0; mf < 4; ++mf) {
+            sc[mf] = __builtin_bit_cast(v4f, pp[mf * 3]);
+            bi[mf] = __builtin_bit_cast(v4f, pp[mf * 3 + 1]);
+        }
+        const v4i z = {0, 0, 0, 0};
+#pragma unroll
+        for (int j = 0; j < TN; ++j) {
+            v4i* tp = tile + (j * 16 + frow) * CPR + ((cg / 16) ^ frow);
+            const v4i rs = *tp;
+            v4i o;
+            o.x = (int)chain_elt_pack(acc[0][j], z, bi[0], sc[0], (unsigned)rs.x, lo_s8, res_lo, a);
+            o.y = (int)chain_elt_pack(acc[1][j], z, bi[1], sc[1], (unsigned)rs.y, lo_s8, res_lo, a);
+            o.z = (int)chain_elt_pack(acc[2][j], z, bi[2], sc[2], (unsigned)rs.z, lo_s8, res_lo, a);
+            o.w = (int)chain_elt_pack(acc[3][j], z, bi[3], sc[3], (unsigned)rs.w, lo_s8, res_lo, a);
+            *tp = o;
+        }
+    }
+    SABER_TL(3);
+    asm volatile("s_waitcnt lgkmcnt(0)" ::: "memory");
+    __builtin_amdgcn_s_barrier();
+
+    {
+        char* yg = (char*)a.y1;
+        constexpr int NIT = NPX * CPR / (64 * NW);
+#pragma unroll
+        for (int it = 0; it < NIT; ++it) {
+            const int L = it * (64 * NW) + tid;
+            const int px = L / CPR, c = (L % CPR) ^ (px & 15);
+            bool ok;
+            const int p = pix(px, ok);
+            if (ok) *(v4i*)(yg + (size_t)p * K1 + c * 16) = tile[L];
+        }
+    }
+    v4i b2[KS2][TN];
+#pragma unroll
+    for (int j = 0; j < TN; ++j)
+#pragma unroll
+        for (int ks = 0; ks < KS2; ++ks) b2[ks][j] = tile[(j * 16 + frow) * CPR + ((ks * 4 + fq) ^ frow)];
+    SABER_TL(4);
+
+    constexpr int G2S = TH + T0 + T1;
+    {
+        v4i acc[TN];
+        const int cg = wave * 16 + fq * 4;
+        const float lo2 = a.relu2 ? 0.f : -3.0e38f;
+        const float off2 = a.out_u8_2 ? 0.f : 128.f;
+        const unsigned xm2 = a.out_u8_2 ? 0u : 0x80808080u;
+        const v4i* pp = prm2 + (cg / 4) * 3;
+#pragma unroll
+        for (int j = 0; j < TN; ++j) acc[j] = pp[2];
+#pragma unroll
+        for (int s = 0; s < T2; ++s) {
+#pragma unroll
+            for (int j = 0; j < TN; ++j) acc[j] = mma_step(ring[(G2S + s) % R], b2[s][j], acc[j]);
+            if (G2S + s + R < TOT) ring[(G2S + s) % R] = step(G2S + s + R);
+        }
+#pragma unroll
+        for (int j = 0; j < TN; ++j) {
+            const unsigned o = chain_out_pack(acc[j], v4i{0, 0, 0, 0}, __builtin_bit_cast(v4f, pp[1]), __builtin_bit_cast(v4f, pp[0]), lo2, off2, xm2);
+            bool ok;
+            const int p = pix(j * 16 + frow, ok);
+            if (ok) *(unsigned*)((char*)a.y2 + (size_t)p * K2 + cg) = o;
+        }
+    }
+    SABER_TL(5);
+    SABER_TL_FLUSH();
+}
+
+hipError_t launch_conv_chain_head_c128(const ChainHeadKArgs& h, int rows, hipStream_t s) {
+    const ChainKArgs& a = h.c;
+    if (a.M <= 0 || a.tiles_per_img <= 0 || a.N <= 0 || !a.zero || !h.hstream || !h.hprm || a.s0 != 1) return hipErrorInvalidValue;
+    const dim3 block(512), grid(a.tiles_per_img * a.N);
+    if (rows == 2) hipLaunchKernelGGL((conv_chain_head_c128_kernel<2>), grid, block, 0, s, h);
+    else if (rows == 1) hipLaunchKernelGGL((conv_chain_head_c128_kernel<1>), grid, block, 0, s, h);
+    else return hipErrorInvalidValue;
+    return hipGetLastError();
+}
+
+}
diff --git a/anakin_amd/csrc/kernels.h b/anakin_amd/csrc/kernels.h
--- a/anakin_amd/csrc/kernels.h
+++ b/anakin_amd/csrc/kernels.h
@@ -129,6 +129,13 @@
 };
 bool conv1x1_chain_ok(int c1, int k1, int k2);
 hipError_t launch_conv1x1_chain(const ChainKArgs& a, int c1, int k1, int k2, int rows, int waves, int split, int with3x3, hipStream_t s);
+struct ChainHeadKArgs {
+    ChainKArgs c;
+    const void* hstream;
+    const void* hprm;
+    int hin_u8, hrelu_a, hrelu_b;
+};
+hipError_t launch_conv_chain_head_c128(const ChainHeadKArgs& a, int rows, hipStream_t s);
 hipError_t launch_conv_chain_coop(const CoopKArgs& a, hipStream_t s);
 
 struct StageBlk {
diff --git a/anakin_amd/lib.py b/anakin_amd/lib.py
--- a/anakin_amd/lib.py
+++ b/anakin_amd/lib.py
@@ -20,7 +20,7 @@
     "saber_hip_conv2d_create_pair", "saber_hip_conv2d_run_pair", "saber_hip_conv2d_autotune_pair",
     "saber_hip_net_add_conv_pair",
     "saber_hip_conv2d_chain_create", "saber_hip_conv2d_chain_create3", "saber_hip_conv2d_chain_create3_pair", "saber_hip_conv2d_chain_destroy", "saber_hip_conv2d_chain_run",
-    "saber_hip_conv2d_chain_run3",
+    "saber_hip_conv2d_chain_run3", "saber_hip_conv2d_chain_create3_head", "saber_hip_conv2d_chain_run3_head", "saber_hip_conv2d_chain_has_head",
     "saber_hip_conv2d_chain_set_tile", "saber_hip_conv2d_chain_get_tile",
     "saber_hip_conv2d_stage_create", "saber_hip_conv2d_stage_destroy", "saber_hip_conv2d_stage_run", "saber_hip_conv2d_stage_create_tail", "saber_hip_conv2d_stage_run_tail",
     "saber_hip_conv2d_stage_create_head", "saber_hip_conv2d_stage_run_head",
@@ -38,7 +38,7 @@
     "saber_hip_transpose_nchw_to_nhwc_f32", "saber_hip_transpose_nhwc_to_nchw_f32",
     "saber_hip_quantize_flat_s8", "saber_hip_eltwise_sum_i8", "saber_hip_eltwise_sum_f32", "saber_hip_relu_f32", "saber_hip_activation_f32", "saber_hip_prelu_f32",
     "saber_hip_pool_out_dim", "saber_hip_pool_out_dim2", "saber_hip_pool2d_i8_nhwc", "saber_hip_pool2d_f32", "saber_hip_pool2d_f32_from_i8", "saber_hip_pool2d_f32_from_i8_q", "saber_hip_fc_run_q", "saber_hip_fc_run_softmax", "saber_hip_softmax_f32",
-    "saber_hip_net_add_pool_f32_from_i8_q", "saber_hip_net_add_fc_q", "saber_hip_net_optimize", "saber_hip_net_num_launches", "saber_hip_net_tensor_unwritten", "saber_hip_net_get_choice", "saber_hip_net_set_choice", "saber_hip_net_stage_blocks", "saber_hip_net_stage_head", "saber_hip_net_time_op_in_pass", "saber_hip_net_status", "saber_hip_net_inject_coop_error", "saber_hip_net_coop_fallbacks", "saber_hip_coop_fallbacks_total",
+    "saber_hip_net_add_pool_f32_from_i8_q", "saber_hip_net_add_fc_q", "saber_hip_net_optimize", "saber_hip_net_num_launches", "saber_hip_net_tensor_unwritten", "saber_hip_net_get_choice", "saber_hip_net_set_choice", "saber_hip_net_stage_blocks", "saber_hip_net_stage_head", "saber_hip_net_chain_head", "saber_hip_net_set_chain_head", "saber_hip_net_time_op_in_pass", "saber_hip_net_status", "saber_hip_net_inject_coop_error", "saber_hip_net_coop_fallbacks", "saber_hip_coop_fallbacks_total",
     "saber_hip_net_create", "saber_hip_net_add_tensor", "saber_hip_net_add_conv", "saber_hip_net_add_fc",
     "saber_hip_net_add_quantize", "saber_hip_net_add_dequantize", "saber_hip_net_add_transpose_in_f32", "saber_hip_net_add_eltwise_i8",
     "saber_hip_net_add_eltwise_f32", "saber_hip_net_add_pool_i8", "saber_hip_net_add_pool_f32",
@@ -127,6 +127,9 @@
     lib.saber_hip_conv2d_chain_run.argtypes = [P, P, P, P, P, P]
     lib.saber_hip_conv2d_chain_create3_pair.argtypes = [P, P, P, P, C.POINTER(P)]
     lib.saber_hip_conv2d_chain_run3.argtypes = [P, P, P, P, P, P, P]
+    lib.saber_hip_conv2d_chain_create3_head.argtypes = [P, P, P, P, P, C.POINTER(P)]
+    lib.saber_hip_conv2d_chain_run3_head.argtypes = [P, P, P, P, P]
+    lib.saber_hip_conv2d_chain_has_head.argtypes = [P, I]
     lib.saber_hip_conv2d_chain_set_tile.argtypes = [P, I]
     lib.saber_hip_conv2d_chain_get_tile.argtypes = [P]
     lib.saber_hip_conv2d_stage_create.argtypes = [C.POINTER(P), I, C.POINTER(P)]
@@ -175,6 +178,8 @@
     lib.saber_hip_net_optimize.argtypes = [P, I]
     lib.saber_hip_net_stage_blocks.argtypes = [P, I]
     lib.saber_hip_net_stage_head.argtypes = [P, I]
+    lib.saber_hip_net_chain_head.argtypes = [P, I]
+    lib.saber_hip_net_set_chain_head.argtypes = [P, I, I]
     lib.saber_hip_net_status.argtypes = [P]
     lib.saber_hip_net_inject_coop_error.argtypes = [P]
     lib.saber_hip_net_coop_fallbacks.argtypes = [P]
diff --git a/anakin_amd/saber.py b/anakin_amd/saber.py
--- a/anakin_amd/saber.py
+++ b/anakin_amd/saber.py
@@ -339,10 +339,12 @@
 
 class SaberConvChain:
 
-    def __init__(self, a, b, conv3x3=None, pair_b=None):
-        self.a, self.b, self.c3, self.b2 = a, b, conv3x3, pair_b
-        self.h = C.c_void_p()
-        if pair_b is not None:
+    def __init__(self, a, b, conv3x3=None, pair_b=None, head=None):
+        self.a, self.b, self.c3, self.b2, self.head = a, b, conv3x3, pair_b, head
+        self.h = C.c_void_p()
+        if head is not None:
+            L.check(L.load().saber_hip_conv2d_chain_create3_head(head[0].h, head[1].h, conv3x3.h, a.h, b.h, C.byref(self.h)))
+        elif pair_b is not None:
             L.check(L.load().saber_hip_conv2d_chain_create3_pair(conv3x3.h, a.h, b.h, pair_b.h, C.byref(self.h)))
         elif conv3x3 is None:
             L.check(L.load().saber_hip_conv2d_chain_create(a.h, b.h, C.byref(self.h)))
@@ -352,6 +354,13 @@
     def dispatch(self, x, res, ya, yb=None, yc=None):
         L.check(L.load().saber_hip_conv2d_chain_run3(self.h, _p(x), _p(res), _p(ya), _p(yb), _p(yc), _stream()))
         return ya, yb
+
+    def dispatch_head(self, x_pair, ya, yb):
+        L.check(L.load().saber_hip_conv2d_chain_run3_head(self.h, _p(x_pair), _p(ya), _p(yb), _stream()))
+        return ya, yb
+
+    def has_head(self, tn=0):
+        return bool(L.load().saber_hip_conv2d_chain_has_head(self.h, int(tn)))
 
     def set_tile(self, tn):
         L.check(L.load().saber_hip_conv2d_chain_set_tile(self.h, tn))
@@ -1031,6 +1040,29 @@
                 ch[p] = (ch[p] | (1 << 29)) if on else (ch[p] & ~(1 << 29))
         self.set_choices(ch)
 
+    def chain_head_sites(self):
+        lib = L.load()
+        out = []
+        for i in range(self.num_ops()):
+            p = int(lib.saber_hip_net_chain_head(self.h, i))
+            if p >= 0:
+                out.append((p, i))
+        return out
+
+    def chain_heads(self):
+        ch = self.choices()
+        return [(p, i) for p, i in self.chain_head_sites() if (ch[p] >> 28) & 1]
+
+    def select_chain_heads(self, on, form=None):
+        ch = self.choices()
+        for p, i in self.chain_head_sites():
+            ch[p] = (ch[p] | (1 << 28)) if on else (ch[p] & ~(1 << 28))
+            if on:
+                led = (ch[i] >> 24) & 15 if (ch[i] >> 29) & 1 else 0
+                code = int(form) if form is not None else (led if led in (5, 6) else 6)
+                ch[i] = (ch[i] & ~(15 << 24)) | (1 << 29) | (code << 24)
+        self.set_choices(ch)
+
     def time_ops(self, iters=20):
         out = (C.c_float * self.num_ops())()
         L.check(L.load().saber_hip_net_time_ops(self.h, _stream(), iters, out))
diff --git a/anakin_amd/workloads.py b/anakin_amd/workloads.py
--- a/anakin_amd/workloads.py
+++ b/anakin_amd/workloads.py
@@ -297,7 +297,7 @@
 
 
 def build_int8_net(model, scales, batch, hw=224, fuse=True, chain=2, stage=True, stem_pair=True, head_pair=False, shared_device=False,
-                   fc_softmax=True, absorb_pool=True, separable=False, inverted=False, fire=False, before_finalize=None, **legacy):
+                   chain_head=True, fc_softmax=True, absorb_pool=True, separable=False, inverted=False, fire=False, before_finalize=None, **legacy):
     from . import lib as L
     from . import saber as S
     legacy.pop("cxx_optimize", None)
@@ -383,7 +383,7 @@
         net.gpooled = net.optimize(128) if absorb_pool else 0
         net.stem_paired = net.optimize(512) if stem_pair else 0
         net.chained = net.optimize(16 | (32 if int(chain) >= 2 else 0) | (256 if int(chain) >= 2 and stage else 0) |
-                                   (1024 if int(chain) >= 2 and head_pair else 0)) if chain else 0
+                                   (1024 if int(chain) >= 2 and head_pair else 0) | (131072 if int(chain) >= 2 and chain_head else 0)) if chain else 0
         net.fc_softmaxed = net.optimize(4096) if fc_softmax else 0
     if before_finalize is not None:
         before_finalize(net)
diff --git a/include/saber_hip.h b/include/saber_hip.h
--- a/include/saber_hip.h
+++ b/include/saber_hip.h
@@ -86,6 +86,10 @@
 int saber_hip_conv2d_chain_create3(saber_hip_conv_t* conv3x3, saber_hip_conv_t* a, saber_hip_conv_t* b, saber_hip_chain_t** out);
 int saber_hip_conv2d_chain_create3_pair(saber_hip_conv_t* conv3x3, saber_hip_conv_t* a, saber_hip_conv_t* pair_a, saber_hip_conv_t* pair_b,
                                         saber_hip_chain_t** out);
+int saber_hip_conv2d_chain_create3_head(const saber_hip_conv_t* pair_a, const saber_hip_conv_t* pair_b, saber_hip_conv_t* conv3x3, saber_hip_conv_t* a,
+                                        saber_hip_conv_t* b, saber_hip_chain_t** out);
+int saber_hip_conv2d_chain_run3_head(saber_hip_chain_t* chain, const void* x_pair, void* y_a, void* y_b, saber_hip_stream_t stream);
+int saber_hip_conv2d_chain_has_head(const saber_hip_chain_t* chain, int tn);
 void saber_hip_conv2d_chain_destroy(saber_hip_chain_t* chain);
 int saber_hip_conv2d_chain_run(saber_hip_chain_t* chain, const void* x, const void* res, void* y_a, void* y_b,
                                saber_hip_stream_t stream);
@@ -261,6 +265,7 @@
 #define SABER_HIP_NET_SEPARABLE 16384
 #define SABER_HIP_NET_INVERTED_RESIDUAL 32768
 #define SABER_HIP_NET_FIRE 65536
+#define SABER_HIP_NET_CHAIN_HEAD 131072
 int saber_hip_net_optimize(saber_hip_net_t* net, int flags);
 int saber_hip_net_coop_fallbacks(const saber_hip_net_t* net);
 int saber_hip_coop_fallbacks_total(void);
@@ -268,6 +273,8 @@
 int saber_hip_net_inject_coop_error(saber_hip_net_t* net);
 int saber_hip_net_stage_blocks(const saber_hip_net_t* net, int index);
 int saber_hip_net_stage_head(const saber_hip_net_t* net, int index);
+int saber_hip_net_chain_head(const saber_hip_net_t* net, int index);
+int saber_hip_net_set_chain_head(saber_hip_net_t* net, int index, int on);
 int saber_hip_net_num_launches(const saber_hip_net_t* net);
 int saber_hip_net_tensor_unwritten(const saber_hip_net_t* net, int id);
 int saber_hip_net_add_softmax(saber_hip_net_t* net, int rows, int cols, int in_id, int out_id);
diff --git a/integration/mi355x/framework/mi355x_net_planner.h b/integration/mi355x/framework/mi355x_net_planner.h
--- a/integration/mi355x/framework/mi355x_net_planner.h
+++ b/integration/mi355x/framework/mi355x_net_planner.h
@@ -82,7 +82,9 @@
         const bool stem_pair = env_on("SABER_MI355X_NET_STEM_PAIR", true);
         const bool head_pair = env_on("SABER_MI355X_NET_HEAD_PAIR", false);
         const bool fc_softmax = env_on("SABER_MI355X_NET_FC_SOFTMAX", true);
+        const bool chain_head = env_on("SABER_MI355X_NET_CHAIN_HEAD", true);
         if (ok) ok = saber_hip_net_optimize(n, 255 | (stage ? 256 : 0) | (stem_pair ? 512 : 0) | (head_pair ? 1024 : 0) | (fc_softmax ? 4096 : 0) |
+                                               (chain_head ? SABER_HIP_NET_CHAIN_HEAD : 0) |
                                                (plan.shared_device ? SABER_HIP_NET_SHARED_DEVICE : 0) |
                                                (MI355XNetPlanDefaults::reproducible_fp32() ? SABER_HIP_NET_REPRODUCIBLE_FP32 : 0)) >= 0;
         if (ok) ok = saber_hip_net_finalize(n) == SABER_HIP_OK;
```

Measured after the change: 40210, median of 6. Within noise of the previous version (+0.9%).
